# dmMaze/comic-text-detector

Hardware: NVIDIA H100
Metric: pages/sec @1024x1024 synthetic (higher is better)
Workload: dtype fp16

## Files before the change

### comic-text-detector_b200/csrc/engine.h

```cpp
#pragma once
#include <cuda.h>
#include <cuda_runtime.h>
#include <stdint.h>

#include <math.h>

#include <algorithm>
#include <array>
#include <condition_variable>
#include <deque>
#include <map>
#include <mutex>
#include <optional>
#include <string>
#include <thread>
#include <tuple>
#include <vector>

#include "kernels.h"

using ctd::ConvTcPlan;
using ctd::ConvEndsPlan;
using ctd::NmsWorkspace;
using ctd::PFN_encodeTiled;

struct ArenaLayout {
  size_t det, cnt, nl, lb, ls, lc, a_bytes, refined, blocks, blocks_stride, rec_off, lines_off, dist_off, total;
};

struct BlockSection {
  size_t rec_off, lines_off, dist_off, stride;
};
inline BlockSection block_section_layout() {
  auto al = [](size_t v) { return (v + 255) / 256 * 256; };
  BlockSection b;
  b.rec_off = 64;
  b.lines_off = b.rec_off + al(size_t(CTD_MAX_BLOCKS) * sizeof(ctd_block));
  b.dist_off = b.lines_off + al(size_t(CTD_MAX_BLOCKS) * 32);
  b.stride = b.dist_off + al(size_t(CTD_MAX_BLOCK_DIST) * 8);
  return b;
}

struct Letterbox {
  int unpad_h, unpad_w;
  float ratio_x, ratio_y;
};
inline bool letterbox_of(int ih, int iw, int net_h, int net_w, Letterbox& lb) {
  if (ih < 1 || iw < 1 || net_h < 1 || net_w < 1) return false;
  const double r = std::min(double(net_h) / ih, double(net_w) / iw);
  lb.unpad_w = int(nearbyint(iw * r));
  lb.unpad_h = int(nearbyint(ih * r));
  if (lb.unpad_w < 1 || lb.unpad_h < 1 || lb.unpad_w > net_w || lb.unpad_h > net_h) return false;
  lb.ratio_x = float(double(iw) / double(lb.unpad_w));
  lb.ratio_y = float(double(ih) / double(lb.unpad_h));
  return true;
}

struct PagesHead {
  size_t det, cnt, lb, ls, lc, masks;
};
PagesHead pages_head(int n);

struct JobPage {
  int ih, iw;
  float ratio_x, ratio_y;
  size_t off;
  char* section;
};

struct PipeJob {
  int slot = 0, refine_mode = 0;
  char* results_host = nullptr;
  PagesHead head{};
  size_t refined = 0;
  std::vector<JobPage> pages;
  size_t total = 0;
  const uint8_t* d_img = nullptr;
  uint8_t* d_mask = nullptr;
  uint8_t* d_ref = nullptr;
  uint8_t* d_aux = nullptr;
  uint8_t* d_blocks = nullptr;
  size_t blocks_bytes = 0;
  int keep_undetected = 0;
  int textheight = 0;
  int results_on_device = 0;
};

struct ctd_handle;
template <bool kPinned>
struct GrowBuf {
  uint8_t* p = nullptr;
  size_t cap = 0;
  int grow(ctd_handle* h, size_t bytes, std::optional<cudaStream_t> sync, size_t headroom = 4);
  void release();
};
using DevBuf = GrowBuf<false>;
using PinnedBuf = GrowBuf<true>;

struct Slot {
  uint8_t* d_stage_in = nullptr;
  uint8_t* d_stage_out = nullptr;
  cudaEvent_t ev_in_done = nullptr, ev_in_free = nullptr, ev_out_ready = nullptr, ev_out_done = nullptr;
  cudaEvent_t ev_post_done = nullptr;
  bool busy = false;
  bool full = false;
  bool crops = false, on_device = false, collected = false;
  int state = 0;
  int rc = 0;
  std::string err;
  char* pinned = nullptr;
  DevBuf pg_in, pg_res, pg_aux;
  ctd::PageGeom* h_pg_tab = nullptr;
  ctd::PageGeom* d_pg_tab = nullptr;
  std::vector<ctd_page_entry> dev_pages;
  std::vector<ctd_region> crop_plan;
  std::vector<int32_t> crop_first;
  std::vector<size_t> crop_base;
  DevBuf d_crop;
  PinnedBuf h_crop;
  size_t crop_px_off = 0, crop_bytes = 0;

  void start(bool want_crops, bool want_on_device) {
    crops = want_crops;
    on_device = want_on_device;
    collected = false;
  }
  void release();
};

struct RefineJob {
  std::vector<ctd::RefineWin> wins;
  std::vector<ctd::RefineChunk> chunks;
  size_t total_px = 0;
  void add(int x1, int y1, int x2, int y2, size_t page_off, int iw, int ih);
  size_t table_bytes() const;
};

struct RegionJob {
  std::vector<ctd::RegionDev> regs;
  std::vector<ctd::RegionTile> tiles;
  size_t out_bytes = 0;
  int add(const ctd_region* plan, int n, long long page_off, int ih, int iw, long long out_base);
  size_t table_bytes() const;
  void write_tables(char* dst) const;
};

struct ShapePlan {
  std::vector<ConvTcPlan> tc;
  std::vector<ConvEndsPlan> ends;
  cudaGraphExec_t graph = nullptr;
  int launches = 0;
};
struct ctd_handle {
  ctd_config cfg{};
  std::vector<ctd_op> ops;
  std::vector<ctd_bufdesc> bufs;
  std::vector<std::array<float, 7>> detect_prm;
  std::string err;
  cudaStream_t stream = nullptr;
  cudaEvent_t ev0 = nullptr, ev1 = nullptr, tev0 = nullptr, tev1 = nullptr;
  std::vector<cudaEvent_t> op_events;
  PFN_encodeTiled enc = nullptr;
  char* d_blob = nullptr;
  size_t blob_bytes = 0;
  std::vector<void*> d_buf;
  std::vector<void*> d_buf16;
  char* d_wsplit = nullptr;
  std::vector<size_t> wsplit_off;
  int elem = 2;
  uint8_t* d_pages = nullptr;
  float* d_blks = nullptr;
  float* d_mask = nullptr;
  uint8_t* d_mask_u8 = nullptr;
  size_t results_bytes = 0;
  float* d_lines = nullptr;
  uint8_t* d_bitmap = nullptr;
  float* d_det = nullptr;
  int* d_det_count = nullptr;
  int32_t* d_labels = nullptr;
  int32_t* d_nlabels = nullptr;
  int32_t* d_ccl_scratch = nullptr;
  void* d_segrep_scratch = nullptr;
  DevBuf refine_scratch;
  DevBuf cc_scratch;
  DevBuf io_scratch;
  int16_t* d_line_boxes = nullptr;
  float* d_line_scores = nullptr;
  int32_t* d_line_count = nullptr;
  void* d_nms_ws = nullptr;
  NmsWorkspace nms{};
  std::map<std::tuple<int, int, int>, ShapePlan> plans;
  cudaStream_t copy_in = nullptr, copy_out = nullptr;
  Slot slot[2];
  bool overlap = false;
  cudaStream_t side = nullptr, side2 = nullptr;
  cudaEvent_t ev_fork = nullptr, ev_join = nullptr, ev_fork2 = nullptr, ev_join2 = nullptr;
  cudaEvent_t ev_xjoin = nullptr;
  std::vector<char> db_ancestor;
  ArenaLayout layout{};
  cudaStream_t post = nullptr;
  size_t pipe_pinned_cap = 0;
  std::thread pipe_thread;
  std::mutex pipe_mu;
  std::condition_variable pipe_cv, pipe_done_cv;
  std::deque<PipeJob> pipe_queue;
  bool pipe_quit = false;
  int host_threads = 4;
  size_t pg_gather_off = 0;
  cudaStream_t dev_out = nullptr;
  DevBuf pg_cc;
  DevBuf post_refine;
  int n = 0, ph = 0, pw = 0;
  int last_launches = 0;
  bool have_forward = false;
};


int ctd_fail(ctd_handle* h, int code, const char* fmt, ...);
int prepare_forward(ctd_handle* h, int32_t n, int32_t ph, int32_t pw, ShapePlan** out);
int enqueue_forward(ctd_handle* h, int32_t n, int32_t ph, int32_t pw, ShapePlan& sp);
int ensure_pipeline(ctd_handle* h);
int stage_phase_a(ctd_handle* h, Slot& s, const uint8_t* pages, bool pages_on_device, int n, int ph, int pw,
                  ShapePlan& sp, void* results_host);
int cc_device(ctd_handle* h, const uint8_t* d_img, int ih, int iw, int stats_cap, int32_t** d_stats, int32_t* n_labels);
int launch_refine(ctd_handle* h, const RefineJob& job, const uint8_t* d_img, const uint8_t* d_mask, int refine_mode,
                  uint8_t* d_out, cudaStream_t st, DevBuf& scratch, char* pinned);
int ctd_collect_full(ctd_handle* h, int slot);
void ctd_pipeline_shutdown(ctd_handle* h);
```

### comic-text-detector_b200/csrc/kernels.h

```cpp
#pragma once
#include <cuda.h>
#include <cuda_fp16.h>
#include <cuda_runtime.h>
#include <stdint.h>

#include "../../include/ctd_b200.h"

namespace ctd {

constexpr int kMaxTaps = 9;

constexpr float kSplitLoScale = 2048.0f;
constexpr float kSplitLoUnscale = 1.0f / 2048.0f;
constexpr int kMaxPhases = 4;

struct ConvGeom {
  int n_img;
  int gh, gw;
  int dst_h, dst_w;
  int out_mul;
  int n_phase;
  int taps;
  int cin_total;
  int k_total;
  int n_src;
  int src_c[CTD_MAX_SRC];
  int src_cstride[CTD_MAX_SRC];
  int src_h, src_w;
  int in_stride;
  int8_t tap_dy[kMaxPhases][kMaxTaps];
  int8_t tap_dx[kMaxPhases][kMaxTaps];
  int cout, cout_pad;
  int dst_cstride, dst_coff;
  int act, residual;
};

void fill_conv_geom_taps(ConvGeom& g, int kind, int ksize, int stride);

struct alignas(64) ConvTcParams {
  CUtensorMap a_map[CTD_MAX_SRC][4];
  CUtensorMap b_map;
  CUtensorMap d_map[kMaxPhases];
  ConvGeom g;
  int kb_elems;
  int src_kblocks[CTD_MAX_SRC];
  int tiles_x, tiles_y;
  int8_t tap_map[kMaxPhases][kMaxTaps];
  __half* dst;
  int dst_map_cols;
  const float* bias;
  float* blks;
  int blks_rows_per_img;
  int level_row0;
  float det_stride;
  float anchor_wh[6];
  int nc;
  int split;
  int split_img_off;
  int split_row_off;
};
static_assert(sizeof(ConvTcParams) <= 4096, "ConvTcParams: kernel parameters are limited to 4 KB");

struct ConvTcPlan {
  ConvTcParams p;
  int block_n;
  int tile_h;
  dim3 grid;
  size_t smem_bytes;
};

typedef CUresult (*PFN_encodeTiled)(CUtensorMap*, CUtensorMapDataType, cuuint32_t, void*, const cuuint64_t*,
                                    const cuuint64_t*, const cuuint32_t*, const cuuint32_t*, CUtensorMapInterleave,
                                    CUtensorMapSwizzle, CUtensorMapL2promotion, CUtensorMapFloatOOBfill);

const char* conv_tc_plan(ConvTcPlan& plan, PFN_encodeTiled enc, const ConvGeom& g, const void* const src_ptr[],
                         const int src_coff[], const void* w16, const float* bias, __half* dst, int split = 0);
cudaError_t conv_tc_launch(const ConvTcPlan& plan, cudaStream_t s);
cudaError_t conv_tc_init();

enum { CTD_END_NONE = 0, CTD_END_STEM = 1, CTD_END_SEG = 2 };
struct alignas(64) ConvEndsParams {
  CUtensorMap a_map;
  CUtensorMap b_map;
  CUtensorMap d_map;
  int n_img, gh, gw;
  int tiles_x, tiles_y;
  const float* bias;
  float* mask_f32;
  uint8_t* mask_u8;
};
struct ConvEndsPlan {
  ConvEndsParams p;
  int kind = CTD_END_NONE;
  dim3 grid;
  size_t smem_bytes;
};
const char* conv_ends_plan_stem(ConvEndsPlan& plan, PFN_encodeTiled enc, const uint8_t* pages, int n, int ph, int pw,
                                const void* w16, const float* bias, __half* dst, int dst_cstride, int dst_coff,
                                int cout, int act);
const char* conv_ends_plan_seg(ConvEndsPlan& plan, PFN_encodeTiled enc, const __half* src, int src_cstride,
                               int src_coff, int src_c, int n, int gh, int gw, const void* w16, float* mask_f32,
                               uint8_t* mask_u8);
cudaError_t conv_ends_launch(const ConvEndsPlan& plan, cudaStream_t s);
cudaError_t conv_ends_init();

struct ConvSimtParams {
  ConvGeom g;
  const void* src[CTD_MAX_SRC];
  const void* w;
  const float* bias;
  void* dst;
  float* blks;
  int blks_rows_per_img, level_row0, nc;
  float det_stride;
  float anchor_wh[6];
};
template <typename T>
cudaError_t conv_simt_launch(const ConvSimtParams& p, cudaStream_t s);

template <typename T>
cudaError_t stem_launch(const uint8_t* pages, int n, int h, int w, const float* wgt ,
                        const float* bias, T* dst, int dst_cstride, int dst_coff, int cout, int act, cudaStream_t s);
cudaError_t split_planes_launch(const float* src, __half* hi, __half* lo, size_t npix, int c, int cstride,
                                cudaStream_t s);
template <typename T>
cudaError_t avgpool2_launch(const T* src, int n, int h, int w, int c, int src_cstride, T* dst, int dst_cstride,
                            cudaStream_t s);
template <typename T>
cudaError_t sppf_pool_launch(T* buf, int n, int h, int w, int c, int cstride, cudaStream_t s);
template <typename T>
cudaError_t upsample2_launch(const T* src, int n, int h, int w, int c, int src_cstride, T* dst, int dst_cstride,
                             cudaStream_t s);
template <typename T>
cudaError_t seg_tail_launch(const T* src, int n, int h, int w, int c, int cstride, const float* wgt ,
                            float* mask_f32, uint8_t* mask_u8, cudaStream_t s);
template <typename T>
cudaError_t db_tail_launch(const T* src, int n, int h, int w, int cstride, const float* params, float* lines,
                           uint8_t* bitmap, float db_thresh, cudaStream_t s);

struct NmsWorkspace {
  float* cand;
  int* cand_count;
  int* cand_total;
  float* sorted;
  unsigned long long* mask;
  int cap;
};
cudaError_t nms_launch(const float* blks, int n, int rows, int nc, float conf, float iou, NmsWorkspace& ws,
                       float* det , int* det_count, cudaStream_t s);
constexpr int kNmsLaunches = 5;
size_t nms_workspace_bytes(int n, int cap);
void nms_workspace_bind(NmsWorkspace& ws, void* base, int n, int cap);

cudaError_t ccl_launch(const uint8_t* img, int n, int h, int w, int32_t* labels, int32_t* scratch ,
                       int32_t* n_labels, cudaStream_t s);
constexpr int kCclLaunches = 8;
cudaError_t ccl_stats_launch(const int32_t* labels, int h, int w, int32_t* stats, int cap, cudaStream_t s);

size_t segrep_scratch_bytes(int n, int h, int w, int max_cand);
cudaError_t segrep_launch(const uint8_t* bitmap, const float* pred, size_t pred_page_stride, const int* Lf, int n, int h,
                          int w, int max_cand, float unclip_ratio, void* scratch, int16_t* boxes, float* scores,
                          int* n_contours, cudaStream_t s);
constexpr int kSegrepLaunches = 15;
cudaError_t binarize_launch(const float* pred, size_t count, float thresh, uint8_t* bitmap, cudaStream_t s);

cudaError_t resize_linear_u8_launch(const uint8_t* src, int sh, int sw, size_t src_pitch, int channels, uint8_t* dst,
                                    int dh, int dw, int canvas_h, int canvas_w, cudaStream_t s);
struct PageGeom {
  long long src_off, dst_off;
  int ih, iw, unpad_h, unpad_w, row0, pad;
};
cudaError_t letterbox_batch_launch(const uint8_t* src, const PageGeom* d_tab, int n, uint8_t* dst, int net_h, int net_w,
                                   cudaStream_t s);
cudaError_t backproject_batch_launch(const uint8_t* mask, int net_h, int net_w, const PageGeom* d_tab, int n,
                                     int total_rows, uint8_t* dst, cudaStream_t s);

struct GatherPage {
  const uint8_t* src;
  long long sh, sw, sc;
  long long dst_off;
  int ih, iw, row0, fast;
};
cudaError_t gather_pages_launch(const GatherPage* d_tab, int n, int total_rows, uint8_t* dst, cudaStream_t s);

struct RefineWin {
  int x1, y1, x2, y2;
  long long off;
  long long page_off;
  int pitch;
};
struct RefineChunk { int win, y0, x0, rows; };
constexpr int kRefineChunkPx = 8192;
__host__ __device__ constexpr int refine_rows_per_chunk(int rw) {
  return kRefineChunkPx / rw >= 8 ? (kRefineChunkPx / rw) & ~3 : (kRefineChunkPx / rw > 0 ? kRefineChunkPx / rw : 1);
}
size_t refine_scratch_bytes(size_t total_px, size_t n_chunks);
size_t refine_mk_state_bytes(int n_wins);
cudaError_t refine_mk_launch(const uint8_t* d_img, const uint8_t* d_mask, const RefineWin* d_wins, int n_wins,
                             const RefineChunk* d_chunks, int n_chunks, int n_multi_chunks, void* d_state, size_t total_px,
                             void* scratch, int refine_mode, uint8_t* d_out, cudaStream_t s);

constexpr int kRegionTilePx = 256;
struct RegionDev {
  long long offset;
  long long page_off;
  int out_h, out_w;
  int warp_w, bw0;
  int rotate, ih, iw, pad;
  double m[9];
};
struct RegionTile { int region, first; };
cudaError_t warp_regions_launch(const uint8_t* d_pages, const RegionDev* d_regs, const RegionTile* d_tiles, int n_tiles,
                                uint8_t* d_out, cudaStream_t s);

}
```

### comic-text-detector_b200/csrc/pipeline.cu

```cuda
#include <cuda.h>
#include <cuda_runtime.h>
#include <math.h>
#include <stdint.h>
#include <string.h>

#include <algorithm>
#include <thread>
#include <vector>

#include "engine.h"

using namespace ctd;

#define CK(expr)                                                                                      \
  do {                                                                                                \
    cudaError_t _e = (expr);                                                                          \
    if (_e != cudaSuccess) return ctd_fail(h, CTD_E_CUDA, "%s: %s (%s:%d)", #expr, cudaGetErrorString(_e), __FILE__, __LINE__); \
  } while (0)

namespace {
inline void norm_slice(int& lo, int& hi, int n) {
  if (lo < 0) lo = std::max(lo + n, 0);
  if (hi < 0) hi = std::max(hi + n, 0);
  lo = std::min(lo, n);
  hi = std::min(hi, n);
  if (hi < lo) hi = lo;
}
}

void RefineJob::add(int x1, int y1, int x2, int y2, size_t page_off, int iw, int ih) {
  norm_slice(x1, x2, iw);
  norm_slice(y1, y2, ih);
  const size_t a = (x2 > x1 && y2 > y1) ? size_t(x2 - x1) * (y2 - y1) : 0;
  if (a == 0) return;
  const int wi = int(wins.size());
  const int rw = x2 - x1, rh = y2 - y1;
  const int rows_per = refine_rows_per_chunk(rw);
  for (int y0 = 0; y0 < rh; y0 += rows_per)
    for (int x0 = 0; x0 < rw; x0 += kRefineChunkPx) chunks.push_back(RefineChunk{wi, y0, x0, std::min(rows_per, rh - y0)});
  wins.push_back(RefineWin{x1, y1, x2, y2, (long long)total_px, (long long)page_off, iw});
  total_px = (total_px + a + 3) / 4 * 4;
}
size_t RefineJob::table_bytes() const {
  auto al = [](size_t v) { return (v + 255) / 256 * 256; };
  return al(wins.size() * sizeof(RefineWin)) + al(chunks.size() * sizeof(RefineChunk));
}

int launch_refine(ctd_handle* h, const RefineJob& job, const uint8_t* d_img, const uint8_t* d_mask, int refine_mode,
                  uint8_t* d_out, cudaStream_t st, DevBuf& scratch, char* pinned) {
  if (job.wins.empty()) return CTD_OK;
  auto al = [](size_t v) { return (v + 255) / 256 * 256; };
  const size_t tb = job.table_bytes();
  const size_t sb = refine_mk_state_bytes(int(job.wins.size()));
  if (int rc = scratch.grow(h, tb + sb + refine_scratch_bytes(job.total_px, job.chunks.size()), st, 2)) return rc;
  char* base = reinterpret_cast<char*>(scratch.p);
  const size_t wb = al(job.wins.size() * sizeof(RefineWin));
  std::vector<char> local;
  char* stage = pinned;
  if (!stage) { local.resize(tb); stage = local.data(); }
  memcpy(stage, job.wins.data(), job.wins.size() * sizeof(RefineWin));
  int n_multi = 0;
  {
    RefineChunk* hc = reinterpret_cast<RefineChunk*>(stage + wb);
    const size_t nc = job.chunks.size();
    size_t tail = nc;
    for (size_t i = 0; i < nc;) {
      size_t j = i;
      while (j < nc && job.chunks[j].win == job.chunks[i].win) ++j;
      if (j - i > 1) {
        for (size_t k = i; k < j; ++k) hc[n_multi++] = job.chunks[k];
      } else {
        hc[--tail] = job.chunks[i];
      }
      i = j;
    }
  }
  CK(cudaMemcpyAsync(base, stage, tb, cudaMemcpyHostToDevice, st));
  if (!pinned) CK(cudaStreamSynchronize(st));
  CK(refine_mk_launch(d_img, d_mask, reinterpret_cast<const RefineWin*>(base), int(job.wins.size()),
                      reinterpret_cast<const RefineChunk*>(base + wb), int(job.chunks.size()), n_multi, base + tb,
                      job.total_px, base + tb + sb, refine_mode, d_out, st));
  return CTD_OK;
}

extern "C" int ctd_refine_mask(ctd_handle* h, const uint8_t* img, const uint8_t* mask, int32_t ih, int32_t iw,
                               const int32_t* windows, int32_t n_win, int32_t refine_mode, uint8_t* out) {
  if (!h || !img || !mask || !out || (n_win > 0 && !windows)) return CTD_E_INVALID;
  if (ih < 1 || iw < 1) return ctd_fail(h, CTD_E_SHAPE, "bad image size");
  CK(cudaSetDevice(h->cfg.device));
  RefineJob job;
  for (int i = 0; i < n_win; ++i) job.add(windows[4 * i], windows[4 * i + 1], windows[4 * i + 2], windows[4 * i + 3], 0, iw, ih);
  const size_t px = size_t(ih) * iw, pxa = (px + 255) / 256 * 256;
  if (int rc = h->io_scratch.grow(h, pxa * 5 + 1024, h->stream)) return rc;
  uint8_t* d_img = h->io_scratch.p;
  uint8_t* d_mask = d_img + pxa * 3;
  uint8_t* d_out = d_mask + pxa;
  CK(cudaMemcpyAsync(d_img, img, px * 3, cudaMemcpyHostToDevice, h->stream));
  CK(cudaMemcpyAsync(d_mask, mask, px, cudaMemcpyHostToDevice, h->stream));
  CK(cudaMemsetAsync(d_out, 0, pxa, h->stream));
  if (int rc = launch_refine(h, job, d_img, d_mask, refine_mode, d_out, h->stream, h->refine_scratch, nullptr))
    return rc;
  CK(cudaMemcpyAsync(out, d_out, px, cudaMemcpyDeviceToHost, h->stream));
  CK(cudaStreamSynchronize(h->stream));
  return CTD_OK;
}

namespace {
struct PageIn {
  const float* det; int n_det;
  const int16_t* line_boxes; const float* line_scores; int n_lines;
  const uint8_t* mask; int im_w, im_h;
  float ratio_x, ratio_y;
};

PageIn page_in(const char* res, const PagesHead& head, int i, const JobPage& p, const uint8_t* mask) {
  PageIn in;
  in.det = reinterpret_cast<const float*>(res + head.det) + size_t(i) * 300 * 6;
  in.n_det = std::min(std::max(reinterpret_cast<const int32_t*>(res + head.cnt)[i], 0), 300);
  in.line_boxes = reinterpret_cast<const int16_t*>(res + head.lb) + size_t(i) * 1000 * 8;
  in.line_scores = reinterpret_cast<const float*>(res + head.ls) + size_t(i) * 1000;
  in.n_lines = std::min(std::max(reinterpret_cast<const int32_t*>(res + head.lc)[i], 0), 1000);
  in.mask = mask; in.im_w = p.iw; in.im_h = p.ih; in.ratio_x = p.ratio_x; in.ratio_y = p.ratio_y;
  return in;
}

int host_group_page(const PageIn& in, char* section, const BlockSection& L, std::vector<int32_t>& win_out) {
  std::vector<int32_t> bxy(size_t(in.n_det) * 4), bcls(size_t(in.n_det));
  for (int i = 0; i < in.n_det; ++i) {
    const float* d = in.det + 6 * i;
    bxy[4 * i + 0] = int32_t(d[0] * in.ratio_x);
    bxy[4 * i + 1] = int32_t(d[1] * in.ratio_y);
    bxy[4 * i + 2] = int32_t(d[2] * in.ratio_x);
    bxy[4 * i + 3] = int32_t(d[3] * in.ratio_y);
    bcls[i] = int32_t(d[5]);
  }
  std::vector<int32_t> lines;
  lines.reserve(size_t(in.n_lines) * 8);
  for (int i = 0; i < in.n_lines; ++i) {
    if (!(in.line_scores[i] > 0.6f)) continue;
    const int16_t* b = in.line_boxes + 8 * i;
    for (int k = 0; k < 4; ++k) {
      lines.push_back(int32_t(double(b[2 * k]) * double(in.ratio_x)));
      lines.push_back(int32_t(double(b[2 * k + 1]) * double(in.ratio_y)));
    }
  }
  ctd_page_blocks* hdr = reinterpret_cast<ctd_page_blocks*>(section);
  ctd_block* rec = reinterpret_cast<ctd_block*>(section + L.rec_off);
  int32_t* lout = reinterpret_cast<int32_t*>(section + L.lines_off);
  double* dout = reinterpret_cast<double*>(section + L.dist_off);
  int32_t nb = 0;
  int rc = ctd_group_output(bxy.data(), bcls.data(), in.n_det, lines.data(), int32_t(lines.size() / 8), in.im_w, in.im_h, in.mask,
                            1, rec, CTD_MAX_BLOCKS, lout, CTD_MAX_BLOCKS, dout, CTD_MAX_BLOCK_DIST, &nb);
  hdr->flags = 0;
  if (rc == CTD_E_CAPACITY) {
    std::vector<double> big(size_t(CTD_MAX_BLOCKS) * CTD_MAX_BLOCKS / 4);
    rc = ctd_group_output(bxy.data(), bcls.data(), in.n_det, lines.data(), int32_t(lines.size() / 8), in.im_w, in.im_h, in.mask, 1,
                          rec, CTD_MAX_BLOCKS, lout, CTD_MAX_BLOCKS, big.data(), int32_t(big.size()), &nb);
    if (rc == CTD_OK)
      for (int i = 0; i < nb; ++i) { rec[i].n_dist = 0; rec[i].dist_off = 0; }
    hdr->flags |= 1;
  }
  if (rc != CTD_OK) { hdr->n_blocks = 0; hdr->n_lines = 0; hdr->n_dist = 0; hdr->flags |= 2; return rc; }
  hdr->n_blocks = nb;
  int32_t tl = 0, td = 0;
  for (int i = 0; i < nb; ++i) { tl += rec[i].n_lines; td += rec[i].n_dist; }
  hdr->n_lines = tl;
  hdr->n_dist = td;
  win_out.resize(size_t(nb) * 4);
  for (int i = 0; i < nb; ++i) {
    const int32_t* xy = rec[i].xyxy;
    const int64_t w = int64_t(xy[2]) - xy[0], hh = int64_t(xy[3]) - xy[1];
    const int64_t pad = int64_t(nearbyint((double(std::max(hh, w)) * 0.25 + double(std::min(hh, w)) * 0.75) / 16.0));
    win_out[4 * i + 0] = int32_t(std::max<int64_t>(0, xy[0] - pad));
    win_out[4 * i + 1] = int32_t(std::max<int64_t>(0, xy[1] - pad));
    win_out[4 * i + 2] = int32_t(std::min<int64_t>(in.im_w - 1, xy[2] + pad));
    win_out[4 * i + 3] = int32_t(std::min<int64_t>(in.im_h - 1, xy[3] + pad));
  }
  return CTD_OK;
}

template <typename F>
void for_each_page(int n, int threads, F fn) {
  const int nthreads = std::max(1, std::min(n, threads));
  if (nthreads == 1) {
    for (int i = 0; i < n; ++i) fn(i);
    return;
  }
  std::vector<std::thread> th;
  for (int t = 0; t < nthreads; ++t)
    th.emplace_back([&, t] { for (int i = t; i < n; i += nthreads) fn(i); });
  for (auto& x : th) x.join();
}

__global__ void undetected_prep_kernel(uint8_t* __restrict__ mask, const uint8_t* __restrict__ refined,
                                       uint8_t* __restrict__ thr, size_t n) {
  const size_t i = blockIdx.x * size_t(blockDim.x) + threadIdx.x;
  if (i >= n) return;
  uint8_t m = mask[i];
  if (refined[i] > 30) { m = 0; mask[i] = 0; }
  thr[i] = m > 30 ? 255 : 0;
}
__global__ void or_kernel(uint8_t* __restrict__ dst, const uint8_t* __restrict__ src, size_t n) {
  const size_t i = blockIdx.x * size_t(blockDim.x) + threadIdx.x;
  if (i < n) dst[i] |= src[i];
}

struct Planes {
  const uint8_t* img;
  uint8_t *mask, *ref, *ref2, *thr;
  size_t total;
};

int refine_undetected(ctd_handle* h, const std::vector<JobPage>& pages, const Planes& pl, int refine_mode,
                      cudaStream_t st, DevBuf& cc, DevBuf& refine_scratch, char* pinned, size_t pinned_cap) {
  auto al = [](size_t v) { return (v + 255) / 256 * 256; };
  const int n = int(pages.size());
  const size_t total_px = pl.total;
  undetected_prep_kernel<<<unsigned((total_px + 255) / 256), 256, 0, st>>>(pl.mask, pl.ref, pl.thr, total_px);
  CK(cudaGetLastError());
  size_t max_px = 0;
  std::vector<int> cap(static_cast<size_t>(n));
  std::vector<size_t> stats_off(static_cast<size_t>(n));
  for (int i = 0; i < n; ++i) max_px = std::max(max_px, size_t(pages[i].ih) * pages[i].iw);
  const size_t o_scr = al(max_px * 4);
  size_t o = o_scr + al(max_px * 12);
  for (int i = 0; i < n; ++i) {
    cap[size_t(i)] = ((pages[i].ih + 1) / 2) * ((pages[i].iw + 1) / 2) + 2;
    stats_off[size_t(i)] = o;
    o += al(size_t(cap[size_t(i)]) * 5 * 4);
  }
  const size_t o_nl = o;
  if (int rc = cc.grow(h, o_nl + al(size_t(n) * 4), st)) return rc;
  uint8_t* base = cc.p;
  int32_t* d_labels = reinterpret_cast<int32_t*>(base);
  int32_t* d_scr = reinterpret_cast<int32_t*>(base + o_scr);
  int32_t* d_nl = reinterpret_cast<int32_t*>(base + o_nl);
  for (int i = 0; i < n; ++i) {
    const JobPage& p = pages[size_t(i)];
    int32_t* d_stats = reinterpret_cast<int32_t*>(base + stats_off[size_t(i)]);
    CK(ccl_launch(pl.thr + p.off, 1, p.ih, p.iw, d_labels, d_scr, d_nl + i, st));
    CK(ccl_stats_launch(d_labels, p.ih, p.iw, d_stats, cap[size_t(i)], st));
  }
  std::vector<int32_t> n_lab(static_cast<size_t>(n));
  CK(cudaMemcpyAsync(n_lab.data(), d_nl, size_t(n) * 4, cudaMemcpyDeviceToHost, st));
  CK(cudaStreamSynchronize(st));
  std::vector<std::vector<int32_t>> stats(static_cast<size_t>(n));
  for (int i = 0; i < n; ++i) {
    stats[size_t(i)].resize(size_t(std::max(n_lab[size_t(i)], 0)) * 5);
    if (n_lab[size_t(i)] > 0)
      CK(cudaMemcpyAsync(stats[size_t(i)].data(), base + stats_off[size_t(i)], stats[size_t(i)].size() * 4,
                         cudaMemcpyDeviceToHost, st));
  }
  CK(cudaStreamSynchronize(st));
  const BlockSection bs = block_section_layout();
  RefineJob rj2;
  for (int i = 0; i < n; ++i) {
    const JobPage& p = pages[size_t(i)];
    const int nb = reinterpret_cast<const ctd_page_blocks*>(p.section)->n_blocks;
    const ctd_block* rec = reinterpret_cast<const ctd_block*>(p.section + bs.rec_off);
    bool first_valid = true;
    for (int li = 0; li < n_lab[size_t(i)]; ++li) {
      const int32_t* s5 = &stats[size_t(i)][size_t(li) * 5];
      if (!(s5[4] > 50)) continue;
      if (first_valid) { first_valid = false; continue; }
      const int64_t bb[4] = {s5[0], s5[1], int64_t(s5[0]) + s5[2], int64_t(s5[1]) + s5[3]};
      int64_t score = -1;
      for (int b = 0; b < nb; ++b) {
        const int32_t* q = rec[b].xyxy;
        const int64_t x1 = std::max<int64_t>(q[0], bb[0]), y1 = std::max<int64_t>(q[1], bb[1]);
        const int64_t x2 = std::min<int64_t>(q[2], bb[2]), y2 = std::min<int64_t>(q[3], bb[3]);
        const int64_t a = (y2 < y1 || x2 < x1) ? -1 : (y2 - y1) * (x2 - x1);
        if (a > score) score = a;
      }
      if (double(score) / double(s5[2]) / double(s5[3]) < 0.5) {
        int32_t xy[4] = {int32_t(bb[0]), int32_t(bb[1]), int32_t(bb[2]), int32_t(bb[3])}, w4[4];
        const int64_t w = bb[2] - bb[0], hh = bb[3] - bb[1];
        const int64_t pad = int64_t(nearbyint((double(std::max(hh, w)) * 0.25 + double(std::min(hh, w)) * 0.75) / 16.0));
        w4[0] = int32_t(std::max<int64_t>(0, xy[0] - pad)); w4[1] = int32_t(std::max<int64_t>(0, xy[1] - pad));
        w4[2] = int32_t(std::min<int64_t>(p.iw - 1, xy[2] + pad)); w4[3] = int32_t(std::min<int64_t>(p.ih - 1, xy[3] + pad));
        rj2.add(w4[0], w4[1], w4[2], w4[3], p.off, p.iw, p.ih);
      }
    }
  }
  if (!rj2.wins.empty()) {
    CK(cudaMemsetAsync(pl.ref2, 0, total_px, st));
    char* stage = rj2.table_bytes() <= pinned_cap ? pinned : nullptr;
    if (int rc = launch_refine(h, rj2, pl.img, pl.mask, refine_mode, pl.ref2, st, refine_scratch, stage)) return rc;
    or_kernel<<<unsigned((total_px + 255) / 256), 256, 0, st>>>(pl.ref, pl.ref2, total_px);
    CK(cudaGetLastError());
  }
  return CTD_OK;
}

int phase_c(ctd_handle* h, const std::vector<JobPage>& pages, const std::vector<std::vector<int32_t>>& wins,
            const Planes& pl, int refine_mode, bool keep_undetected, cudaStream_t st, DevBuf& refine_scratch,
            DevBuf& cc, char* pinned, size_t pinned_cap) {
  RefineJob rj;
  for (size_t i = 0; i < pages.size(); ++i)
    for (size_t k = 0; k + 3 < wins[i].size(); k += 4)
      rj.add(wins[i][k], wins[i][k + 1], wins[i][k + 2], wins[i][k + 3], pages[i].off, pages[i].iw, pages[i].ih);
  char* stage = rj.table_bytes() <= pinned_cap ? pinned : nullptr;
  if (int rc = launch_refine(h, rj, pl.img, pl.mask, refine_mode, pl.ref, st, refine_scratch, stage)) return rc;
  if (!keep_undetected) return CTD_OK;
  return refine_undetected(h, pages, pl, refine_mode, st, cc, refine_scratch, pinned, pinned_cap);
}
}

extern "C" int ctd_results_layout(ctd_handle* h, ctd_results_layout_t* out) {
  if (!h || !out) return CTD_E_INVALID;
  const ArenaLayout& L = h->layout;
  out->max_batch = h->cfg.max_batch; out->max_h = h->cfg.max_h; out->max_w = h->cfg.max_w; out->reserved = 0;
  out->total_bytes = L.total;
  out->mask_u8 = 0; out->det = L.det; out->det_count = L.cnt; out->n_labels = L.nl;
  out->line_boxes = L.lb; out->line_scores = L.ls; out->line_count = L.lc;
  out->phase_a_bytes = L.a_bytes;
  out->mask_refined = L.refined; out->blocks = L.blocks; out->blocks_stride = L.blocks_stride;
  out->blk_records_off = L.rec_off; out->blk_lines_off = L.lines_off; out->blk_dist_off = L.dist_off;
  return CTD_OK;
}

PagesHead pages_head(int n) {
  auto al = [](size_t v) { return (v + 255) / 256 * 256; };
  const size_t nb = size_t(n);
  PagesHead hd;
  hd.det = 0;
  hd.cnt = hd.det + al(nb * 300 * 6 * 4);
  hd.lb = hd.cnt + al(nb * 4);
  hd.ls = hd.lb + al(nb * 1000 * 8 * 2);
  hd.lc = hd.ls + al(nb * 1000 * 4);
  hd.masks = hd.lc + al(nb * 4);
  return hd;
}

extern "C" int ctd_pages_plan(ctd_page_entry* pages, int32_t n, int32_t net_h, int32_t net_w, size_t* input_bytes,
                              size_t* results_bytes) {
  if (!input_bytes || !results_bytes || n < 0 || (n > 0 && !pages)) return CTD_E_INVALID;
  if (net_h < 64 || net_w < 64 || net_h % 64 || net_w % 64) return CTD_E_SHAPE;
  auto al = [](size_t v) { return (v + 255) / 256 * 256; };
  const PagesHead hd = pages_head(n);
  size_t total = 0;
  for (int i = 0; i < n; ++i) {
    Letterbox lb;
    if (!letterbox_of(pages[i].ih, pages[i].iw, net_h, net_w, lb)) return CTD_E_SHAPE;
    pages[i].unpad_h = lb.unpad_h;
    pages[i].unpad_w = lb.unpad_w;
    pages[i].page_off = int64_t(total * 3);
    pages[i].mask_off = int64_t(hd.masks + total);
    total += al(size_t(pages[i].ih) * size_t(pages[i].iw));
  }
  const size_t stride = al(block_section_layout().stride);
  const size_t blocks = hd.masks + 2 * total;
  for (int i = 0; i < n; ++i) {
    pages[i].refined_off = pages[i].mask_off + int64_t(total);
    pages[i].blocks_off = int64_t(blocks + size_t(i) * stride);
  }
  *input_bytes = total * 3;
  *results_bytes = blocks + size_t(n) * stride;
  return CTD_OK;
}

static int plan_page_regions(const char* section, const BlockSection& bs, int iw, int ih, int textheight,
                             std::vector<ctd_region>& plan, size_t* bytes) {
  const ctd_page_blocks* hdr = reinterpret_cast<const ctd_page_blocks*>(section);
  const ctd_block* rec = reinterpret_cast<const ctd_block*>(section + bs.rec_off);
  const int32_t* quads = reinterpret_cast<const int32_t*>(section + bs.lines_off);
  std::vector<ctd_region_line> lines;
  lines.reserve(size_t(std::max(hdr->n_lines, 0)));
  for (int b = 0; b < hdr->n_blocks; ++b)
    for (int k = 0; k < rec[b].n_lines; ++k) {
      ctd_region_line l{};
      const int32_t* q = quads + size_t(rec[b].line_off + k) * 8;
      for (int j = 0; j < 8; ++j) l.quad[j] = double(q[j]);
      l.language = rec[b].language;
      l.vertical = rec[b].vertical ? 1 : 0;
      l.font_size = rec[b].font_size;
      lines.push_back(l);
    }
  plan.resize(lines.size());
  *bytes = 0;
  if (lines.empty()) return CTD_OK;
  return ctd_region_plan(lines.data(), int32_t(lines.size()), iw, ih, textheight, plan.data(), bytes);
}

static int run_batch(ctd_handle* h, const PipeJob& job) {
  Slot& s = h->slot[job.slot];
  const int n = int(job.pages.size());
  CK(cudaEventSynchronize(s.ev_out_done));
  char* res = job.results_host;
  const BlockSection bs = block_section_layout();
  std::vector<std::vector<int32_t>> wins(static_cast<size_t>(n));
  std::vector<int> prc(size_t(n), CTD_OK);
  const bool crops = job.textheight > 0;
  std::vector<std::vector<ctd_region>> plans(crops ? size_t(n) : 0);
  std::vector<size_t> plan_bytes(size_t(n), 0);
  std::vector<int> crc(size_t(n), CTD_OK);
  for_each_page(n, h->host_threads, [&](int i) {
    const JobPage& p = job.pages[size_t(i)];
    const uint8_t* mask = reinterpret_cast<const uint8_t*>(res + job.head.masks + p.off);
    prc[size_t(i)] = host_group_page(page_in(res, job.head, i, p, mask), p.section, bs, wins[size_t(i)]);
    if (crops && prc[size_t(i)] == CTD_OK)
      crc[size_t(i)] = plan_page_regions(p.section, bs, p.iw, p.ih, job.textheight, plans[size_t(i)],
                                         &plan_bytes[size_t(i)]);
  });
  for (int i = 0; i < n; ++i)
    if (prc[size_t(i)] != CTD_OK) return ctd_fail(h, prc[size_t(i)], "group_output failed on page %d of the batch", i);
  for (int i = 0; i < n; ++i)
    if (crc[size_t(i)] != CTD_OK)
      return ctd_fail(h, crc[size_t(i)], "ctd_region_plan refused page %d of the batch (%dx%d, textheight %d)", i,
                      job.pages[size_t(i)].ih, job.pages[size_t(i)].iw, job.textheight);
  RegionJob rg;
  if (crops) {
    s.crop_plan.clear();
    s.crop_first.assign(size_t(n) + 1, 0);
    s.crop_base.assign(size_t(n) + 1, 0);
    size_t base = 0;
    for (int i = 0; i < n; ++i) {
      const JobPage& pg = job.pages[size_t(i)];
      const std::vector<ctd_region>& p = plans[size_t(i)];
      if (int bad = rg.add(p.data(), int(p.size()), (long long)(pg.off * 3), pg.ih, pg.iw, (long long)base); bad >= 0)
        return ctd_fail(h, CTD_E_INVALID, "malformed crop plan entry %d on page %d of the batch", bad, i);
      s.crop_first[size_t(i)] = int32_t(s.crop_plan.size());
      s.crop_base[size_t(i)] = base;
      for (ctd_region r : p) {
        r.offset += int64_t(base);
        s.crop_plan.push_back(r);
      }
      base += plan_bytes[size_t(i)];
    }
    s.crop_first[size_t(n)] = int32_t(s.crop_plan.size());
    s.crop_base[size_t(n)] = base;
    if (s.crop_plan.size() > size_t(INT32_MAX) || rg.tiles.size() > size_t(INT32_MAX))
      return ctd_fail(h, CTD_E_CAPACITY, "too many crops in one batch");
    s.crop_bytes = base;
    s.crop_px_off = 0;
  }
  cudaStream_t st = h->post;
  CK(cudaStreamWaitEvent(st, s.ev_out_ready, 0));
  if (job.d_blocks)
    CK(cudaMemcpyAsync(job.d_blocks, job.pages[0].section, job.blocks_bytes, cudaMemcpyHostToDevice, st));
  const bool to_host = !job.results_on_device;
  if (!rg.tiles.empty()) {
    const size_t tb = rg.table_bytes(), px = s.crop_bytes;
    if (int rc = s.d_crop.grow(h, tb + px, st)) return rc;
    if (int rc = s.h_crop.grow(h, to_host ? tb + px : tb, st)) return rc;
    uint8_t* d_tab = s.d_crop.p;
    rg.write_tables(reinterpret_cast<char*>(s.h_crop.p));
    CK(cudaMemcpyAsync(d_tab, s.h_crop.p, tb, cudaMemcpyHostToDevice, st));
    const size_t rb = (rg.regs.size() * sizeof(ctd::RegionDev) + 255) / 256 * 256;
    CK(ctd::warp_regions_launch(job.d_img, reinterpret_cast<const ctd::RegionDev*>(d_tab),
                                reinterpret_cast<const ctd::RegionTile*>(d_tab + rb), int(rg.tiles.size()), d_tab + tb,
                                st));
    if (to_host) CK(cudaMemcpyAsync(s.h_crop.p + tb, d_tab + tb, px, cudaMemcpyDeviceToHost, st));
    s.crop_px_off = tb;
  }
  CK(cudaMemsetAsync(job.d_ref, 0, job.total, st));
  const Planes pl{job.d_img, job.d_mask, job.d_ref, job.d_aux, job.d_aux ? job.d_aux + job.total : nullptr, job.total};
  if (int rc = phase_c(h, job.pages, wins, pl, job.refine_mode, job.keep_undetected, st, h->post_refine, h->pg_cc,
                       s.pinned, h->pipe_pinned_cap))
    return rc;
  if (to_host) {
    if (job.keep_undetected) CK(cudaMemcpyAsync(res + job.head.masks, job.d_mask, job.total, cudaMemcpyDeviceToHost, st));
    CK(cudaMemcpyAsync(res + job.refined, job.d_ref, job.total, cudaMemcpyDeviceToHost, st));
  }
  CK(cudaEventRecord(s.ev_post_done, st));
  return CTD_OK;
}

static void pipe_worker(ctd_handle* h) {
  cudaSetDevice(h->cfg.device);
  for (;;) {
    PipeJob job;
    {
      std::unique_lock<std::mutex> lk(h->pipe_mu);
      h->pipe_cv.wait(lk, [&] { return h->pipe_quit || !h->pipe_queue.empty(); });
      if (h->pipe_queue.empty()) return;
      job = std::move(h->pipe_queue.front());
      h->pipe_queue.pop_front();
    }
    const int rc = run_batch(h, job);
    std::string err;
    if (rc != CTD_OK) err = h->err;
    {
      std::lock_guard<std::mutex> lk(h->pipe_mu);
      Slot& s = h->slot[job.slot];
      s.state = rc == CTD_OK ? 2 : 3;
      s.rc = rc;
      s.err = err;
    }
    h->pipe_done_cv.notify_all();
  }
}

static void queue_job(ctd_handle* h, PipeJob&& job) {
  Slot& s = h->slot[job.slot];
  {
    std::lock_guard<std::mutex> lk(h->pipe_mu);
    s.state = 1;
    h->pipe_queue.push_back(std::move(job));
  }
  h->pipe_cv.notify_one();
  s.busy = true;
  s.full = true;
}

static int ensure_full_pipeline(ctd_handle* h) {
  if (int rc = ensure_pipeline(h)) return rc;
  if (h->pipe_thread.joinable()) return CTD_OK;
  int lo = 0, hi = 0;
  CK(cudaDeviceGetStreamPriorityRange(&lo, &hi));
  CK(cudaStreamCreateWithPriority(&h->post, cudaStreamNonBlocking, hi));
  h->pipe_pinned_cap = size_t(h->cfg.max_batch) * (size_t(CTD_MAX_BLOCKS) * sizeof(RefineWin) +
                                                   size_t(CTD_MAX_BLOCKS) * sizeof(RefineChunk) * 8) + (size_t(8) << 20);
  for (Slot& s : h->slot) {
    CK(cudaHostAlloc(reinterpret_cast<void**>(&s.pinned), h->pipe_pinned_cap, cudaHostAllocDefault));
    CK(cudaEventCreateWithFlags(&s.ev_post_done, cudaEventDisableTiming));
  }
  const char* ht = getenv("CTD_HOST_THREADS");
  const unsigned hc = std::thread::hardware_concurrency();
  h->host_threads = ht ? atoi(ht) : int(std::max(1u, std::min(8u, hc ? hc / 2 : 4u)));
  h->pipe_quit = false;
  h->pipe_thread = std::thread(pipe_worker, h);
  return CTD_OK;
}

void ctd_pipeline_shutdown(ctd_handle* h) {
  if (h->pipe_thread.joinable()) {
    {
      std::lock_guard<std::mutex> lk(h->pipe_mu);
      h->pipe_quit = true;
    }
    h->pipe_cv.notify_all();
    h->pipe_thread.join();
  }
  if (h->post) cudaStreamDestroy(h->post);
  h->post = nullptr;
  if (h->dev_out) cudaStreamDestroy(h->dev_out);
  h->dev_out = nullptr;
  h->pg_cc.release();
  h->post_refine.release();
}

extern "C" int ctd_submit_full(ctd_handle* h, int32_t slot, const uint8_t* pages, int32_t n, int32_t ph, int32_t pw,
                               int32_t pages_on_device, int32_t refine_mode, void* results_host) {
  if (!h || !pages || !results_host || slot < 0 || slot > 1) return CTD_E_INVALID;
  if (h->cfg.debug_skip_postproc) return ctd_fail(h, CTD_E_INVALID, "ctd_submit_full needs the full pipeline");
  Slot& s = h->slot[slot];
  if (s.busy) return ctd_fail(h, CTD_E_INVALID, "slot %d has an uncollected submission", slot);
  ShapePlan* sp = nullptr;
  if (int rc = prepare_forward(h, n, ph, pw, &sp)) return rc;
  if (int rc = ensure_full_pipeline(h)) return rc;
  s.start(false, false);
  if (int rc = stage_phase_a(h, s, pages, pages_on_device != 0, n, ph, pw, *sp, results_host)) return rc;
  CK(cudaStreamWaitEvent(h->post, s.ev_out_ready, 0));
  const ArenaLayout& L = h->layout;
  const size_t px = size_t(ph) * pw;
  PipeJob job;
  job.slot = slot; job.refine_mode = refine_mode;
  job.results_host = static_cast<char*>(results_host);
  job.head = PagesHead{L.det, L.cnt, L.lb, L.ls, L.lc, 0};
  job.refined = L.refined;
  for (int i = 0; i < n; ++i)
    job.pages.push_back(JobPage{ph, pw, 1.f, 1.f, size_t(i) * px, job.results_host + L.blocks + size_t(i) * L.blocks_stride});
  job.total = size_t(n) * px;
  job.d_img = pages_on_device ? pages : s.d_stage_in;
  job.d_mask = s.d_stage_out;
  job.d_ref = s.d_stage_out + L.refined;
  job.d_blocks = s.d_stage_out + L.blocks;
  job.blocks_bytes = size_t(n) * L.blocks_stride;
  queue_job(h, std::move(job));
  return CTD_OK;
}

extern "C" int ctd_submit_pages(ctd_handle* h, int32_t slot, const ctd_page_entry* pages, int32_t n, int32_t net_h,
                                int32_t net_w, const uint8_t* input_host, int32_t refine_mode, int32_t keep_undetected,
                                void* results_host) {
  return ctd_submit_pages_regions(h, slot, pages, n, net_h, net_w, input_host, refine_mode, keep_undetected, 0,
                                  results_host);
}

extern "C" int ctd_submit_pages_regions(ctd_handle* h, int32_t slot, const ctd_page_entry* pages, int32_t n,
                                        int32_t net_h, int32_t net_w, const uint8_t* input_host, int32_t refine_mode,
                                        int32_t keep_undetected, int32_t textheight, void* results_host) {
  if (!input_host) return CTD_E_INVALID;
  return ctd_submit_pages_device(h, slot, pages, n, net_h, net_w, input_host, nullptr, refine_mode, keep_undetected,
                                 textheight, 0, results_host);
}

static bool is_device_memory(const void* p, int device) {
  cudaPointerAttributes a{};
  if (cudaPointerGetAttributes(&a, p) != cudaSuccess) {
    cudaGetLastError();
    return false;
  }
  return a.type == cudaMemoryTypeDevice && a.device == device;
}

extern "C" int ctd_submit_pages_device(ctd_handle* h, int32_t slot, const ctd_page_entry* pages, int32_t n,
                                       int32_t net_h, int32_t net_w, const uint8_t* input_host,
                                       const ctd_device_page* dev, int32_t refine_mode, int32_t keep_undetected,
                                       int32_t textheight, int32_t results_on_device, void* results_host) {
  if (!h || !pages || !results_host || slot < 0 || slot > 1 || n < 1) return CTD_E_INVALID;
  if (textheight != 0 && textheight < 2) return ctd_fail(h, CTD_E_INVALID, "textheight %d < 2", textheight);
  if (h->cfg.debug_skip_postproc) return ctd_fail(h, CTD_E_INVALID, "ctd_submit_pages needs the full pipeline");
  Slot& s = h->slot[slot];
  if (s.busy) return ctd_fail(h, CTD_E_INVALID, "slot %d has an uncollected submission", slot);
  if (n > h->cfg.max_batch) return ctd_fail(h, CTD_E_CAPACITY, "batch %d exceeds max_batch %d", n, h->cfg.max_batch);
  std::vector<ctd_page_entry> pg(pages, pages + n);
  size_t in_bytes = 0, res_bytes = 0;
  if (int rc = ctd_pages_plan(pg.data(), n, net_h, net_w, &in_bytes, &res_bytes))
    return ctd_fail(h, rc, "the pages do not letterbox into a %dx%d net input", net_h, net_w);
  if (memcmp(pg.data(), pages, size_t(n) * sizeof(ctd_page_entry)) != 0)
    return ctd_fail(h, CTD_E_INVALID, "the page entries are not the ones ctd_pages_plan returns");
  size_t rows = 0;
  for (int i = 0; i < n; ++i) rows += size_t(pg[size_t(i)].ih);
  if (rows > size_t(INT32_MAX)) return ctd_fail(h, CTD_E_CAPACITY, "the pages of a batch have more than 2^31 rows");
  CK(cudaSetDevice(h->cfg.device));
  int n_dev = 0;
  for (int i = 0; i < n; ++i) {
    if (!dev || !dev[i].data) {
      if (!input_host) return ctd_fail(h, CTD_E_INVALID, "page %d is in neither input_host nor device memory", i);
      continue;
    }
    const ctd_device_page& d = dev[i];
    const int64_t kMaxStride = int64_t(1) << 31;
    if (d.stride_h < 0 || d.stride_w < 0 || d.stride_c < 0 || d.stride_h > kMaxStride || d.stride_w > kMaxStride ||
        d.stride_c > kMaxStride)
      return ctd_fail(h, CTD_E_INVALID, "page %d: strides (%lld, %lld, %lld) out of range [0, 2^31]", i,
                      (long long)d.stride_h, (long long)d.stride_w, (long long)d.stride_c);
    const ctd_page_entry& e = pg[size_t(i)];
    const uint8_t* last = d.data + (e.ih - 1) * d.stride_h + (e.iw - 1) * d.stride_w + 2 * d.stride_c;
    if (!is_device_memory(d.data, h->cfg.device) || !is_device_memory(last, h->cfg.device))
      return ctd_fail(h, CTD_E_INVALID, "page %d (%p) is not device memory of GPU %d", i, (const void*)d.data,
                      h->cfg.device);
    ++n_dev;
  }
  ShapePlan* sp = nullptr;
  if (int rc = prepare_forward(h, n, net_h, net_w, &sp)) return rc;
  if (int rc = ensure_full_pipeline(h)) return rc;
  const ArenaLayout& L = h->layout;
  const PagesHead hd = pages_head(n);
  const size_t total = size_t(pg[0].refined_off - pg[0].mask_off);
  const size_t d2h = size_t(pg[0].refined_off);
  s.start(textheight > 0, results_on_device != 0);
  if (int rc = s.pg_in.grow(h, in_bytes, std::nullopt)) return rc;
  if (int rc = s.pg_res.grow(h, d2h + total, std::nullopt)) return rc;
  if (keep_undetected)
    if (int rc = s.pg_aux.grow(h, 2 * total, std::nullopt)) return rc;
  if (!s.h_pg_tab) {
    h->pg_gather_off = (size_t(h->cfg.max_batch) * sizeof(PageGeom) + 255) / 256 * 256;
    const size_t tab_bytes = h->pg_gather_off + size_t(h->cfg.max_batch) * sizeof(GatherPage);
    CK(cudaHostAlloc(reinterpret_cast<void**>(&s.h_pg_tab), tab_bytes, cudaHostAllocDefault));
    CK(cudaMalloc(reinterpret_cast<void**>(&s.d_pg_tab), tab_bytes));
  }
  PageGeom* tab = s.h_pg_tab;
  GatherPage* gtab = reinterpret_cast<GatherPage*>(reinterpret_cast<char*>(tab) + h->pg_gather_off);
  int row0 = 0, n_gather = 0, gather_rows = 0;
  for (int i = 0; i < n; ++i) {
    const ctd_page_entry& e = pg[size_t(i)];
    tab[i] = PageGeom{e.page_off, e.mask_off - int64_t(hd.masks), e.ih, e.iw, e.unpad_h, e.unpad_w, row0, 0};
    row0 += e.ih;
    if (dev && dev[i].data) {
      const ctd_device_page& d = dev[i];
      gtab[n_gather++] = GatherPage{d.data, (long long)d.stride_h, (long long)d.stride_w, (long long)d.stride_c,
                                    (long long)e.page_off, e.ih, e.iw, gather_rows,
                                    d.stride_c == 1 && d.stride_w == 3 ? 1 : 0};
      gather_rows += e.ih;
    }
  }
  const size_t tab_bytes = n_gather ? h->pg_gather_off + size_t(n_gather) * sizeof(GatherPage) : size_t(n) * sizeof(PageGeom);
  CK(cudaMemcpyAsync(s.d_pg_tab, tab, tab_bytes, cudaMemcpyHostToDevice, h->copy_in));
  if (n_dev == 0) {
    CK(cudaMemcpyAsync(s.pg_in.p, input_host, in_bytes, cudaMemcpyHostToDevice, h->copy_in));
  } else {
    for (int i = 0; i < n;) {
      if (dev[i].data) { ++i; continue; }
      int j = i;
      while (j + 1 < n && !dev[j + 1].data) ++j;
      const size_t lo = size_t(pg[size_t(i)].page_off);
      const size_t hi = size_t(pg[size_t(j)].page_off) + size_t(pg[size_t(j)].ih) * size_t(pg[size_t(j)].iw) * 3;
      CK(cudaMemcpyAsync(s.pg_in.p + lo, input_host + lo, hi - lo, cudaMemcpyHostToDevice, h->copy_in));
      i = j + 1;
    }
  }
  CK(cudaEventRecord(s.ev_in_done, h->copy_in));
  CK(cudaEventRecord(h->ev0, h->stream));
  CK(cudaStreamWaitEvent(h->stream, s.ev_in_done, 0));
  if (n_gather) {
    for (int i = 0; i < n; ++i)
      if (dev[i].data && dev[i].event) CK(cudaStreamWaitEvent(h->stream, static_cast<cudaEvent_t>(dev[i].event), 0));
    CK(gather_pages_launch(reinterpret_cast<const GatherPage*>(reinterpret_cast<const char*>(s.d_pg_tab) +
                                                               h->pg_gather_off),
                           n_gather, gather_rows, s.pg_in.p, h->stream));
  }
  CK(letterbox_batch_launch(s.pg_in.p, s.d_pg_tab, n, h->d_pages, net_h, net_w, h->stream));
  if (int rc = enqueue_forward(h, n, net_h, net_w, *sp)) return rc;
  uint8_t* d_res = s.pg_res.p;
  CK(backproject_batch_launch(h->d_mask_u8, net_h, net_w, s.d_pg_tab, n, row0, d_res + hd.masks, h->stream));
  const size_t nb = size_t(n);
  CK(cudaMemcpyAsync(d_res + hd.det, h->d_mask_u8 + L.det, nb * 300 * 6 * 4, cudaMemcpyDeviceToDevice, h->stream));
  CK(cudaMemcpyAsync(d_res + hd.cnt, h->d_mask_u8 + L.cnt, nb * 4, cudaMemcpyDeviceToDevice, h->stream));
  CK(cudaMemcpyAsync(d_res + hd.lb, h->d_mask_u8 + L.lb, nb * 1000 * 8 * 2, cudaMemcpyDeviceToDevice, h->stream));
  CK(cudaMemcpyAsync(d_res + hd.ls, h->d_mask_u8 + L.ls, nb * 1000 * 4, cudaMemcpyDeviceToDevice, h->stream));
  CK(cudaMemcpyAsync(d_res + hd.lc, h->d_mask_u8 + L.lc, nb * 4, cudaMemcpyDeviceToDevice, h->stream));
  CK(cudaEventRecord(s.ev_out_ready, h->stream));
  CK(cudaStreamWaitEvent(h->copy_out, s.ev_out_ready, 0));
  CK(cudaMemcpyAsync(results_host, d_res, d2h, cudaMemcpyDeviceToHost, h->copy_out));
  CK(cudaEventRecord(s.ev_out_done, h->copy_out));
  PipeJob job;
  job.slot = slot; job.refine_mode = refine_mode;
  job.results_host = static_cast<char*>(results_host);
  job.head = hd;
  job.refined = size_t(pg[0].refined_off);
  for (const ctd_page_entry& e : pg) {
    Letterbox lb;
    letterbox_of(e.ih, e.iw, net_h, net_w, lb);
    job.pages.push_back(JobPage{e.ih, e.iw, lb.ratio_x, lb.ratio_y, size_t(e.mask_off) - hd.masks,
                                job.results_host + e.blocks_off});
  }
  job.total = total;
  job.d_img = s.pg_in.p;
  job.d_mask = d_res + hd.masks;
  job.d_ref = d_res + pg[0].refined_off;
  job.d_aux = keep_undetected ? s.pg_aux.p : nullptr;
  job.keep_undetected = keep_undetected ? 1 : 0;
  job.textheight = textheight;
  job.results_on_device = results_on_device ? 1 : 0;
  if (results_on_device) s.dev_pages = std::move(pg);
  queue_job(h, std::move(job));
  return CTD_OK;
}

int ctd_collect_full(ctd_handle* h, int slot) {
  Slot& s = h->slot[slot];
  int rc;
  {
    std::unique_lock<std::mutex> lk(h->pipe_mu);
    h->pipe_done_cv.wait(lk, [&] { return s.state >= 2; });
    rc = s.rc;
    if (rc != CTD_OK) h->err = s.err;
    s.state = 0;
  }
  s.full = false;
  if (rc != CTD_OK) return rc;
  CK(cudaEventSynchronize(s.ev_post_done));
  s.collected = true;
  return CTD_OK;
}

extern "C" int ctd_collect_device(ctd_handle* h, int32_t slot, void* const* page_dst) {
  if (!h || slot < 0 || slot > 1 || !page_dst) return CTD_E_INVALID;
  const Slot& s = h->slot[slot];
  if (s.busy || !s.collected || !s.on_device)
    return ctd_fail(h, CTD_E_INVALID, "slot %d holds no collected batch with results on the device", slot);
  CK(cudaSetDevice(h->cfg.device));
  const std::vector<ctd_page_entry>& pg = s.dev_pages;
  const int n = int(pg.size());
  for (int i = 0; i < n; ++i)
    if (!page_dst[i] || !is_device_memory(page_dst[i], h->cfg.device))
      return ctd_fail(h, CTD_E_INVALID, "page_dst[%d] (%p) is not device memory of GPU %d", i, page_dst[i],
                      h->cfg.device);
  if (!h->dev_out) CK(cudaStreamCreateWithFlags(&h->dev_out, cudaStreamNonBlocking));
  const uint8_t* d_res = s.pg_res.p;
  const uint8_t* d_px = s.crops ? s.d_crop.p + s.crop_px_off : nullptr;
  for (int i = 0; i < n; ++i) {
    const ctd_page_entry& e = pg[size_t(i)];
    const size_t px = size_t(e.ih) * size_t(e.iw);
    uint8_t* dst = static_cast<uint8_t*>(page_dst[i]);
    CK(cudaMemcpyAsync(dst, d_res + e.mask_off, px, cudaMemcpyDeviceToDevice, h->dev_out));
    CK(cudaMemcpyAsync(dst + px, d_res + e.refined_off, px, cudaMemcpyDeviceToDevice, h->dev_out));
    if (s.crops) {
      const size_t b0 = s.crop_base[size_t(i)], b1 = s.crop_base[size_t(i) + 1];
      if (b1 > b0) CK(cudaMemcpyAsync(dst + 2 * px, d_px + b0, b1 - b0, cudaMemcpyDeviceToDevice, h->dev_out));
    }
  }
  CK(cudaStreamSynchronize(h->dev_out));
  return CTD_OK;
}

extern "C" int ctd_collect_regions(ctd_handle* h, int32_t slot, const ctd_region** plan, int32_t* n_regions,
                                   const int32_t** page_first, const uint8_t** pixels, size_t* bytes) {
  if (!h || slot < 0 || slot > 1 || !plan || !n_regions || !page_first || !pixels || !bytes) return CTD_E_INVALID;
  const Slot& s = h->slot[slot];
  if (s.busy || !s.collected || !s.crops)
    return ctd_fail(h, CTD_E_INVALID, "slot %d holds no collected ctd_submit_pages_regions batch", slot);
  *plan = s.crop_plan.data();
  *n_regions = int32_t(s.crop_plan.size());
  *page_first = s.crop_first.data();
  *bytes = s.crop_bytes;
  *pixels = s.crop_bytes && !s.on_device ? s.h_crop.p + s.crop_px_off : nullptr;
  return CTD_OK;
}

extern "C" int ctd_device_arena(ctd_handle* h, int32_t slot, void** base, void** post_stream) {
  if (!h || slot < 0 || slot > 1 || !base) return CTD_E_INVALID;
  if (!h->slot[slot].d_stage_out)
    return ctd_fail(h, CTD_E_INVALID, "no pipelined submission has been made on this handle");
  *base = h->slot[slot].d_stage_out;
  if (post_stream) *post_stream = h->post;
  return CTD_OK;
}

extern "C" int ctd_detect_page(ctd_handle* h, const uint8_t* page, int32_t ih, int32_t iw, int32_t net_h, int32_t net_w,
                               int32_t refine_mode, int32_t keep_undetected, uint8_t* mask_out, uint8_t* mask_refined_out,
                               ctd_block* blocks, int32_t blocks_cap, int32_t* lines_out, int32_t lines_cap, double* dist_out,
                               int32_t dist_cap, int32_t* n_blocks) {
  if (!h || !page || !mask_out || !mask_refined_out || !n_blocks) return CTD_E_INVALID;
  if (ih < 1 || iw < 1) return ctd_fail(h, CTD_E_SHAPE, "bad page size %dx%d", ih, iw);
  *n_blocks = 0;
  Letterbox geo;
  if (!letterbox_of(ih, iw, net_h, net_w, geo)) return ctd_fail(h, CTD_E_SHAPE, "page does not letterbox into the net input");
  ShapePlan* sp = nullptr;
  if (int rc = prepare_forward(h, 1, net_h, net_w, &sp)) return rc;
  const size_t px = size_t(ih) * iw, pxa = (px + 255) / 256 * 256;
  if (int rc = h->io_scratch.grow(h, pxa * 7 + 1024, h->stream)) return rc;
  uint8_t* d_page = h->io_scratch.p;
  uint8_t* d_mask = d_page + pxa * 3;
  uint8_t* d_ref = d_mask + pxa;
  uint8_t* d_ref2 = d_ref + pxa;
  uint8_t* d_thr = d_ref2 + pxa;
  cudaStream_t st = h->stream;
  CK(cudaEventRecord(h->ev0, st));
  CK(cudaMemcpyAsync(d_page, page, px * 3, cudaMemcpyHostToDevice, st));
  const bool same = ih == net_h && iw == net_w;
  if (same) CK(cudaMemcpyAsync(h->d_pages, d_page, px * 3, cudaMemcpyDeviceToDevice, st));
  else CK(resize_linear_u8_launch(d_page, ih, iw, size_t(iw) * 3, 3, h->d_pages, geo.unpad_h, geo.unpad_w, net_h, net_w, st));
  if (int rc = enqueue_forward(h, 1, net_h, net_w, *sp)) return rc;
  if (same) CK(cudaMemcpyAsync(d_mask, h->d_mask_u8, px, cudaMemcpyDeviceToDevice, st));
  else CK(resize_linear_u8_launch(h->d_mask_u8, geo.unpad_h, geo.unpad_w, size_t(net_w), 1, d_mask, ih, iw, ih, iw, st));
  const PagesHead hd = pages_head(1);
  std::vector<char> rows(hd.masks);
  CK(cudaMemcpyAsync(mask_out, d_mask, px, cudaMemcpyDeviceToHost, st));
  CK(cudaMemcpyAsync(rows.data() + hd.det, h->d_det, 300 * 6 * 4, cudaMemcpyDeviceToHost, st));
  CK(cudaMemcpyAsync(rows.data() + hd.cnt, h->d_det_count, 4, cudaMemcpyDeviceToHost, st));
  CK(cudaMemcpyAsync(rows.data() + hd.lb, h->d_line_boxes, 1000 * 8 * 2, cudaMemcpyDeviceToHost, st));
  CK(cudaMemcpyAsync(rows.data() + hd.ls, h->d_line_scores, 1000 * 4, cudaMemcpyDeviceToHost, st));
  CK(cudaMemcpyAsync(rows.data() + hd.lc, h->d_line_count, 4, cudaMemcpyDeviceToHost, st));
  CK(cudaMemsetAsync(d_ref, 0, pxa, st));
  CK(cudaStreamSynchronize(st));
  const BlockSection L = block_section_layout();
  std::vector<char> section(L.stride);
  const std::vector<JobPage> pages{JobPage{ih, iw, geo.ratio_x, geo.ratio_y, 0, section.data()}};
  std::vector<std::vector<int32_t>> wins(1);
  if (int rc = host_group_page(page_in(rows.data(), hd, 0, pages[0], mask_out), section.data(), L, wins[0]))
    return ctd_fail(h, rc, "group_output failed");
  const ctd_page_blocks* hdr = reinterpret_cast<const ctd_page_blocks*>(section.data());
  const ctd_block* rec = reinterpret_cast<const ctd_block*>(section.data() + L.rec_off);
  const int nb = hdr->n_blocks;
  *n_blocks = nb;
  if (nb > blocks_cap || hdr->n_lines > lines_cap || hdr->n_dist > dist_cap || (nb > 0 && (!blocks || !lines_out)) ||
      (hdr->n_dist > 0 && !dist_out))
    return ctd_fail(h, CTD_E_CAPACITY, "%d blocks / %d lines / %d distances do not fit the output arrays", nb, hdr->n_lines, hdr->n_dist);
  if (nb > 0) {
    memcpy(blocks, rec, size_t(nb) * sizeof(ctd_block));
    memcpy(lines_out, section.data() + L.lines_off, size_t(hdr->n_lines) * 32);
    if (hdr->n_dist > 0) memcpy(dist_out, section.data() + L.dist_off, size_t(hdr->n_dist) * 8);
  }
  const Planes pl{d_page, d_mask, d_ref, d_ref2, d_thr, px};
  if (int rc = phase_c(h, pages, wins, pl, refine_mode, keep_undetected, st, h->refine_scratch, h->cc_scratch, nullptr, 0))
    return rc;
  if (keep_undetected) CK(cudaMemcpyAsync(mask_out, d_mask, px, cudaMemcpyDeviceToHost, st));
  CK(cudaMemcpyAsync(mask_refined_out, d_ref, px, cudaMemcpyDeviceToHost, st));
  CK(cudaStreamSynchronize(st));
  return CTD_OK;
}
```

### comic-text-detector_b200/csrc/refine_mk.cu

```cuda
#include <cuda_runtime.h>
#include <limits.h>
#include <math.h>

#include "kernels.h"

namespace ctd {

namespace {

constexpr int kThreads = 256;
constexpr int kChunkPx = kRefineChunkPx;

struct WinState {
  int hist[4][256];
  unsigned long long xs[12];
  int lo[3], hi[3], otsu_t[3], ncol;
  int nproc, proc_kind[4], proc_neg[4];
  int area0, max1, cnt1, max2;
  int pad[2];
};

struct Ctx {
  const uint8_t* img_all;
  const uint8_t* mask_all;
  uint32_t* out_all;
  const RefineWin* wins;
  const RefineChunk* chunks;
  WinState* st;
  int mode;
  uint16_t* lab;
  uint16_t* roots;
  int* nroots;
  int* P;
  int* acc;
  uint8_t *grey, *predm, *merged, *tmp;
};
constexpr uint16_t kNoLabel = 0xffffu;
static_assert(kChunkPx <= 0xffff, "a chunk-local offset fits 16 bits below kNoLabel");

struct View {
  RefineWin win;
  int w, rw, rh, y0, x0, rows, cols, i0, cnt, aligned;
  const uint8_t* img;
  const uint8_t* mask;
};

__device__ __forceinline__ View view_of(const Ctx& c, int chunk) {
  View v;
  const RefineChunk ch = c.chunks[chunk];
  v.w = ch.win;
  v.win = c.wins[ch.win];
  v.rw = v.win.x2 - v.win.x1;
  v.rh = v.win.y2 - v.win.y1;
  v.y0 = ch.y0;
  v.x0 = ch.x0;
  v.rows = ch.rows;
  v.cols = min(v.rw - ch.x0, kChunkPx);
  v.i0 = ch.y0 * v.rw + ch.x0;
  v.cnt = ch.rows * v.cols;
  v.aligned = (v.i0 & 3) == 0;
  v.img = c.img_all + size_t(v.win.page_off) * 3;
  v.mask = c.mask_all + size_t(v.win.page_off);
  return v;
}

__device__ __forceinline__ int chunk_start(int y, int x, int rw) {
  if (rw > kChunkPx) return y * rw + (x & ~(kChunkPx - 1));
  const int rows_per = refine_rows_per_chunk(rw);
  return (y / rows_per) * rows_per * rw;
}
static_assert((kChunkPx & (kChunkPx - 1)) == 0, "row segments start on multiples of kChunkPx");

__device__ __forceinline__ int uf_find(const int* L, int a) {
  int p = __ldcg(L + a);
  while (p != a) {
    a = p;
    p = __ldcg(L + a);
  }
  return a;
}
__device__ __forceinline__ int uf_find_compress(int* L, int a) {
  const int r = uf_find(L, a);
  while (a != r) {
    const int p = __ldcg(L + a);
    if (p <= r) break;
    atomicMin(&L[a], r);
    a = p;
  }
  return r;
}
__device__ __forceinline__ void uf_union(int* L, int a, int b) {
  bool done;
  do {
    a = uf_find(L, a);
    b = uf_find(L, b);
    if (a < b) {
      const int old = atomicMin(&L[b], a);
      done = old == b;
      b = old;
    } else if (b < a) {
      const int old = atomicMin(&L[a], b);
      done = old == a;
      a = old;
    } else {
      done = true;
    }
  } while (!done);
}

__device__ __forceinline__ void hist_add(int* hist, int bin) {
  const int b0 = __shfl_sync(0xffffffffu, bin, 0);
  if (__all_sync(0xffffffffu, bin == b0)) {
    if ((threadIdx.x & 31) == 0 && bin >= 0) atomicAdd(&hist[bin], 32);
    return;
  }
  if (bin >= 0) atomicAdd(&hist[bin], 1);
}

struct DivW { int d; float inv; bool fast; };
__device__ __forceinline__ DivW make_div(int d, int n) { return DivW{d, __frcp_rn(float(d)), n < (1 << 24)}; }
__device__ __forceinline__ void divmod(int i, const DivW& dv, int& q, int& r) {
  if (dv.fast) {
    q = __float2int_rz(__int2float_rn(i) * dv.inv);
    r = i - q * dv.d;
    if (r < 0) { --q; r += dv.d; } else if (r >= dv.d) { ++q; r -= dv.d; }
  } else {
    q = i / dv.d;
    r = i - q * dv.d;
  }
}

constexpr int kU = 4;
constexpr int kExtWords = (3 * kChunkPx) / 32 + 4;
static_assert(3 * (kChunkPx + 2) / 32 + 2 < kExtWords, "a row segment's halo rectangle fits the shared bit masks");
struct Halo {
  int ystart, xs, ew, ext, off;
};
__device__ __forceinline__ Halo halo_of(const View& v) {
  Halo h;
  h.ystart = v.y0 > 0 ? v.y0 - 1 : 0;
  h.xs = v.x0 > 0 ? v.x0 - 1 : 0;
  h.ew = min(v.x0 + v.cols + 1, v.rw) - h.xs;
  h.ext = (min(v.y0 + v.rows + 1, v.rh) - h.ystart) * h.ew;
  h.off = (v.y0 - h.ystart) * h.ew + v.x0 - h.xs;
  return h;
}
__device__ __forceinline__ unsigned bits_from(const unsigned* M, int pos) {
  if (pos <= -32) return 0u;
  if (pos < 0) return M[0] << (-pos);
  const int w = pos >> 5, sft = pos & 31;
  return __funnelshift_r(M[w], M[w + 1], sft);
}
__device__ __forceinline__ void row_ends(int x, int rw, unsigned& rs, unsigned& re) {
  rs = 0u;
  for (int j = x == 0 ? 0 : rw - x; j < 32; j += rw) rs |= 1u << j;
  int xe = x + 32;
  if (xe >= rw) xe %= rw;
  re = (rs >> 1) | (xe == 0 ? 0x80000000u : 0u);
}
__global__ void __launch_bounds__(kThreads) k_phase0(Ctx c) {
  __shared__ int sh[4][256];
  __shared__ unsigned N60[kExtWords], N127[kExtWords];
  __shared__ unsigned F60[kChunkPx / 32 + 1], F127[kChunkPx / 32 + 1];
  const View v = view_of(c, blockIdx.x);
  for (int i = threadIdx.x; i < 1024; i += kThreads) (&sh[0][0])[i] = 0;
  for (int i = threadIdx.x; i < kExtWords; i += kThreads) { N60[i] = 0u; N127[i] = 0u; }
  __syncthreads();
  uint8_t* grey = c.grey + v.win.off;
  uint8_t* predm = c.predm + v.win.off;
  uint8_t* merged = c.merged + v.win.off;
  const Halo hl = halo_of(v);
  const DivW dv = make_div(hl.ew, 3 * (kChunkPx + 2) + 1);
  for (int e0 = 0; e0 < hl.ext; e0 += kThreads) {
    const int e = e0 + threadIdx.x;
    int mv = 255;
    if (e < hl.ext) {
      int ye, xe;
      divmod(e, dv, ye, xe);
      mv = v.mask[size_t(v.win.y1 + hl.ystart + ye) * v.win.pitch + v.win.x1 + hl.xs + xe];
    }
    const unsigned b60 = __ballot_sync(0xffffffffu, mv <= 60), b127 = __ballot_sync(0xffffffffu, mv <= 127);
    if ((threadIdx.x & 31) == 0 && e < hl.ext) { N60[e >> 5] = b60; N127[e >> 5] = b127; }
  }
  __syncthreads();
  const int ew = hl.ew;
  for (int w = threadIdx.x; w * 32 < v.cnt; w += kThreads) {
    const int p = w * 32 + hl.off;
    int ye, xe;
    divmod(p, dv, ye, xe);
    unsigned rs, re;
    row_ends(hl.xs + xe, v.rw, rs, re);
    F60[w] = bits_from(N60, p) | bits_from(N60, p - ew) | bits_from(N60, p + ew) | (bits_from(N60, p - 1) & ~rs) |
             (bits_from(N60, p + 1) & ~re);
    F127[w] = bits_from(N127, p) | bits_from(N127, p - ew) | bits_from(N127, p + ew) |
              ((bits_from(N127, p - 1) | bits_from(N127, p - ew - 1) | bits_from(N127, p + ew - 1)) & ~rs) |
              ((bits_from(N127, p + 1) | bits_from(N127, p - ew + 1) | bits_from(N127, p + ew + 1)) & ~re);
  }
  __syncthreads();
  const DivW dvw = make_div(v.rw, v.rw * v.rh);
  for (int k0 = 0; k0 < v.cnt; k0 += kThreads * kU) {
    int b[kU], g[kU], r[kU];
#pragma unroll
    for (int u = 0; u < kU; ++u) {
      const int k = k0 + u * kThreads + threadIdx.x;
      b[u] = -1; g[u] = -1; r[u] = -1;
      if (k < v.cnt) {
        int y, x;
        divmod(v.i0 + k, dvw, y, x);
        const size_t gp = size_t(v.win.y1 + y) * v.win.pitch + v.win.x1 + x;
        b[u] = v.img[gp * 3]; g[u] = v.img[gp * 3 + 1]; r[u] = v.img[gp * 3 + 2];
      }
    }
#pragma unroll
    for (int u = 0; u < kU; ++u) {
      const int k = k0 + u * kThreads + threadIdx.x;
      const bool in = k < v.cnt;
      int gr = 0;
      bool core = false;
      if (in) {
        const int i = v.i0 + k;
        gr = (b[u] * 1868 + g[u] * 9617 + r[u] * 4899 + 8192) >> 14;
        grey[i] = (uint8_t)gr;
        predm[i] = ((F60[k >> 5] >> (k & 31)) & 1u) ? 0 : 255;
        merged[i] = 0;
        core = !((F127[k >> 5] >> (k & 31)) & 1u);
      }
      if (k0 + u * kThreads < v.cnt) {
        hist_add(sh[1], b[u]);
        hist_add(sh[2], g[u]);
        hist_add(sh[3], r[u]);
        hist_add(sh[0], core ? gr : -1);
      }
    }
  }
  __syncthreads();
  int* gh = &c.st[v.w].hist[0][0];
  for (int i = threadIdx.x; i < 1024; i += kThreads) {
    const int val = (&sh[0][0])[i];
    if (val) atomicAdd(&gh[i], val);
  }
}

constexpr int kDecideThreads = 64;
__global__ void __launch_bounds__(kDecideThreads) k_decide1(Ctx c) {
  __shared__ int cnt255[256];
  __shared__ int order[256];
  __shared__ double edges[256];
  __shared__ int s_first, s_last, s_total;
  __shared__ int hist_s[4][256];
  WinState& st = c.st[blockIdx.x];
  const RefineWin win = c.wins[blockIdx.x];
  const int n = (win.x2 - win.x1) * (win.y2 - win.y1);
  for (int i = threadIdx.x; i < 1024; i += kDecideThreads) (&hist_s[0][0])[i] = (&st.hist[0][0])[i];
  const int* hist_g = hist_s[0];
  for (int i = threadIdx.x; i < 256; i += kDecideThreads) cnt255[i] = 0;
  __syncthreads();
  if (threadIdx.x == 0) {
    int first = -1, last = -1, total = 0;
    for (int v = 0; v < 256; ++v)
      if (hist_g[v]) { if (first < 0) first = v; last = v; total += hist_g[v]; }
    s_first = first; s_last = last; s_total = total;
  }
  __syncthreads();
  {
    double fe, le;
    if (s_total == 0) { fe = 0.0; le = 1.0; }
    else if (s_first == s_last) { fe = s_first - 0.5; le = s_last + 0.5; }
    else { fe = s_first; le = s_last; }
    const double step = (le - fe) / 255.0;
    for (int i = threadIdx.x; i < 256; i += kDecideThreads) edges[i] = (i == 255) ? le : __dadd_rn(__dmul_rn((double)i, step), fe);
    __syncthreads();
    for (int v = threadIdx.x; v < 256; v += kDecideThreads) {
      if (!hist_g[v]) continue;
      const double a = (double)v;
      const double f = ((a - fe) / (le - fe)) * 255.0;
      int idx = (int)f;
      if (idx == 255) idx = 254;
      if (a < edges[idx]) --idx;
      if (a >= edges[idx + 1] && idx != 254) ++idx;
      atomicAdd(&cnt255[idx], hist_g[v]);
    }
  }
  __syncthreads();
  for (int b = threadIdx.x; b < 255; b += kDecideThreads) {
    int rank = 0;
    const int cb = cnt255[b];
    for (int q = 0; q < 255; ++q) rank += (cnt255[q] > cb) || (cnt255[q] == cb && q < b);
    order[rank] = b;
  }
  __syncthreads();
  if (threadIdx.x == 0) {
    double top[3];
    int nt = 1;
    top[0] = edges[order[0]];
    const double tol = (double)s_total * 0.001;
    for (int j = 1; j < 255; ++j) {
      const double col = edges[order[j]];
      double dmin = 1e300;
      for (int t = 0; t < nt; ++t) dmin = fmin(dmin, fabs(top[t] - col));
      if (dmin > 10.0) top[nt++] = col;
      if (nt >= 3 || (double)cnt255[order[j]] < tol) break;
    }
    st.ncol = nt;
    for (int t = 0; t < nt; ++t) {
      const double c_top = fmin(top[t] + 30.0, 255.0);
      const double c_bot = c_top - 60.0;
      st.lo[t] = (int)fmin(fmax(rint(c_bot), 0.0), 255.0);
      st.hi[t] = (int)fmin(fmax(rint(c_top), 0.0), 255.0);
    }
  }
  if (threadIdx.x >= 32 && threadIdx.x < 35) {
    const int* hh = hist_s[1 + threadIdx.x - 32];
    const double scale = 1.0 / (double)n;
    double mu = 0;
    for (int i = 0; i < 256; ++i) mu = __dadd_rn(mu, __dmul_rn((double)i, (double)hh[i]));
    mu = __dmul_rn(mu, scale);
    double mu1 = 0, q1 = 0, max_sigma = 0;
    int max_val = 0;
    for (int i = 0; i < 256; ++i) {
      const double p_i = __dmul_rn((double)hh[i], scale);
      mu1 = __dmul_rn(mu1, q1);
      q1 = __dadd_rn(q1, p_i);
      const double q2 = 1.0 - q1;
      if (fmin(q1, q2) < 1.1920929e-07 || fmax(q1, q2) > 1.0 - 1.1920929e-07) continue;
      mu1 = __ddiv_rn(__dadd_rn(mu1, __dmul_rn((double)i, p_i)), q1);
      const double mu2 = __ddiv_rn(__dsub_rn(mu, __dmul_rn(q1, mu1)), q2);
      const double dm = __dsub_rn(mu1, mu2);
      const double sigma = __dmul_rn(__dmul_rn(__dmul_rn(q1, q2), dm), dm);
      if (sigma > max_sigma) { max_sigma = sigma; max_val = i; }
    }
    st.otsu_t[threadIdx.x - 32] = max_val;
  }
}

__global__ void __launch_bounds__(kThreads) k_xor(Ctx c) {
  __shared__ unsigned long long sx[12];
  const View v = view_of(c, blockIdx.x);
  const WinState& st = c.st[v.w];
  if (threadIdx.x < 12) sx[threadIdx.x] = 0ull;
  __syncthreads();
  const uint8_t* grey = c.grey + v.win.off;
  const int ncol = st.ncol;
  int lo[3], hi[3], ot[3];
#pragma unroll
  for (int k = 0; k < 3; ++k) { lo[k] = st.lo[k]; hi[k] = st.hi[k]; ot[k] = st.otsu_t[k]; }
  unsigned pos[6], npx = 0;
#pragma unroll
  for (int k = 0; k < 6; ++k) pos[k] = 0u;
  const DivW dv = make_div(v.rw, v.rw * v.rh);
  for (int k0 = 0; k0 < v.cnt; k0 += kThreads * kU) {
    int mk[kU], gr[kU], ch[kU][3];
#pragma unroll
    for (int u = 0; u < kU; ++u) {
      const int k = k0 + u * kThreads + threadIdx.x;
      mk[u] = -1;
      if (k < v.cnt) {
        int y, x;
        divmod(v.i0 + k, dv, y, x);
        const size_t gp = size_t(v.win.y1 + y) * v.win.pitch + v.win.x1 + x;
        mk[u] = v.mask[gp];
        gr[u] = grey[v.i0 + k];
#pragma unroll
        for (int q = 0; q < 3; ++q) ch[u][q] = v.img[gp * 3 + q];
      }
    }
#pragma unroll
    for (int u = 0; u < kU; ++u) {
      if (mk[u] < 0) continue;
      ++npx;
#pragma unroll
      for (int k = 0; k < 3; ++k) {
        const int t = (gr[u] >= lo[k] && gr[u] <= hi[k]) ? 255 : 0;
        pos[k] += (unsigned)(t ^ mk[u]);
        const int t2 = ch[u][k] > ot[k] ? 255 : 0;
        pos[3 + k] += (unsigned)(t2 ^ mk[u]);
      }
    }
  }
#pragma unroll
  for (int k = 0; k < 6; ++k) {
    const bool used = k >= 3 || k < ncol;
    unsigned long long sp = used ? pos[k] : 0ull, sn = used ? 255ull * npx - pos[k] : 0ull;
    for (int o = 16; o > 0; o >>= 1) {
      sp += __shfl_down_sync(0xffffffffu, sp, o);
      sn += __shfl_down_sync(0xffffffffu, sn, o);
    }
    if ((threadIdx.x & 31) == 0) {
      if (sp) atomicAdd(&sx[2 * k], sp);
      if (sn) atomicAdd(&sx[2 * k + 1], sn);
    }
  }
  __syncthreads();
  if (threadIdx.x < 12 && sx[threadIdx.x]) atomicAdd(&c.st[v.w].xs[threadIdx.x], sx[threadIdx.x]);
}

__global__ void k_decide2(Ctx c, int n_wins) {
  const int w = blockIdx.x * blockDim.x + threadIdx.x;
  if (w >= n_wins) return;
  WinState& st = c.st[w];
  const unsigned long long* xs = st.xs;
  unsigned long long best[4];
  int kind[4], neg[4], np_ = 0;
  for (int k = 0; k < st.ncol; ++k) {
    const bool ng = xs[2 * k + 1] < xs[2 * k];
    best[np_] = ng ? xs[2 * k + 1] : xs[2 * k];
    kind[np_] = k; neg[np_] = ng; ++np_;
  }
  int bc = 0, bneg = 0;
  unsigned long long bv = ~0ull;
  for (int ch = 0; ch < 3; ++ch) {
    const bool ng = xs[6 + 2 * ch + 1] < xs[6 + 2 * ch];
    const unsigned long long val = ng ? xs[6 + 2 * ch + 1] : xs[6 + 2 * ch];
    if (val < bv) { bv = val; bc = ch; bneg = ng; }
  }
  best[np_] = bv; kind[np_] = 3 + bc; neg[np_] = bneg; ++np_;
  for (int i = 1; i < np_; ++i) {
    const unsigned long long val = best[i];
    const int kk = kind[i], nn = neg[i];
    int j = i - 1;
    while (j >= 0 && best[j] > val) { best[j + 1] = best[j]; kind[j + 1] = kind[j]; neg[j + 1] = neg[j]; --j; }
    best[j + 1] = val; kind[j + 1] = kk; neg[j + 1] = nn;
  }
  for (int i = 0; i < np_; ++i) { st.proc_kind[i] = kind[i]; st.proc_neg[i] = neg[i]; }
  st.nproc = np_;
  st.area0 = 0; st.max1 = -1; st.cnt1 = 0; st.max2 = -1;
}

constexpr int kLabelThreads = 512;

__device__ __forceinline__ int suf_find(const int* L, int a) {
  int p = L[a];
  while (p != a) {
    a = p;
    p = L[a];
  }
  return a;
}
__device__ __forceinline__ int suf_find_halve(int* L, int a) {
  int p = L[a];
  while (p != a) {
    const int gp = L[p];
    if (gp != p) atomicMin(&L[a], gp);
    a = p;
    p = gp;
  }
  return a;
}
__device__ __forceinline__ void suf_union(int* L, int a, int b) {
  bool done;
  do {
    a = suf_find_halve(L, a);
    b = suf_find_halve(L, b);
    if (a < b) {
      const int old = atomicMin(&L[b], a);
      done = old == b;
      b = old;
    } else if (b < a) {
      const int old = atomicMin(&L[a], b);
      done = old == a;
      a = old;
    } else {
      done = true;
    }
  } while (!done);
}

__global__ void __launch_bounds__(kLabelThreads, 3) k_label_local(Ctx c, int round) {
  __shared__ int Ls[kChunkPx];
  __shared__ unsigned Mw[kChunkPx / 32 + 2];
  __shared__ unsigned Sw[kChunkPx / 32];
  __shared__ unsigned Gw[kChunkPx / 32];
  __shared__ unsigned Bw[kChunkPx / 32];
  __shared__ int s_fg, s_nroot;
  const View v = view_of(c, blockIdx.x);
  WinState& st = c.st[v.w];
  if (round < 4 && round >= st.nproc) return;
  for (int i = threadIdx.x; i < kChunkPx / 32 + 2; i += kLabelThreads) Mw[i] = 0u;
  if (threadIdx.x == 0) { s_fg = 0; s_nroot = 0; }
  __syncthreads();
  uint16_t* lab = c.lab + v.win.off + v.i0;
  uint16_t* roots = c.roots + v.win.off + v.i0;
  int* P = c.P + v.win.off;
  int* acc = c.acc + 4 * v.win.off;
  const int n = v.rw * v.rh;
  int* area = acc; int* gain = acc + n; int* loss = acc + 2 * n; int* maxi = acc + 3 * n;
  const uint8_t* grey = c.grey + v.win.off;
  const uint8_t* merged = c.merged + v.win.off;
  const uint8_t* predm = c.predm + v.win.off;
  int kind = 0, neg = 0, lo = 0, hi = 0, ot = 0;
  if (round < 4) {
    kind = st.proc_kind[round]; neg = st.proc_neg[round];
    if (kind < 3) { lo = st.lo[kind]; hi = st.hi[kind]; } else ot = st.otsu_t[kind - 3];
  }
  const int lane = threadIdx.x & 31;
  const DivW dv = make_div(v.rw, kChunkPx + 1);
  constexpr int kIt = kChunkPx / kLabelThreads;
  if (v.aligned) {
    const uint32_t* mg32 = reinterpret_cast<const uint32_t*>(merged + v.i0);
    const uint32_t* pd32 = reinterpret_cast<const uint32_t*>(predm + v.i0);
    const uint32_t* gr32 = reinterpret_cast<const uint32_t*>(grey + v.i0);
    const int sh = 4 * (lane & 7);
    const unsigned grp = 0xffu << (8 * (lane >> 3));
#pragma unroll 1
    for (int it = 0; it < kChunkPx / (4 * kLabelThreads); ++it) {
      if (it * 4 * kLabelThreads >= v.cnt) break;
      const int k = 4 * (it * kLabelThreads + int(threadIdx.x));
      unsigned fg4 = 0u, g4 = 0u, b4 = 0u;
      if (k < v.cnt) {
        const unsigned m4 = mg32[k >> 2], p4 = pd32[k >> 2];
        unsigned s4 = m4;
        if (round < 4) {
          if (kind < 3) {
            s4 = gr32[k >> 2];
          } else {
            s4 = 0u;
#pragma unroll
            for (int j = 0; j < 4; ++j) {
              if (k + j < v.cnt) {
                int yl, x;
                divmod(k + j, dv, yl, x);
                s4 |= unsigned(v.img[(size_t(v.win.y1 + v.y0 + yl) * v.win.pitch + v.win.x1 + v.x0 + x) * 3 + (kind - 3)]) << (8 * j);
              }
            }
          }
        }
#pragma unroll
        for (int j = 0; j < 4; ++j) {
          if (k + j < v.cnt) {
            const int sbv = int((s4 >> (8 * j)) & 0xffu), mb = int((m4 >> (8 * j)) & 0xffu), pb = int((p4 >> (8 * j)) & 0xffu);
            bool fg;
            if (round == 4) {
              fg = sbv == 0;
            } else {
              const bool t = kind < 3 ? (sbv >= lo && sbv <= hi) : (sbv > ot);
              fg = neg ? !t : t;
            }
            const bool un = fg && mb == 0;
            fg4 |= unsigned(fg) << j;
            g4 |= unsigned(un && pb != 0) << j;
            b4 |= unsigned(un && pb == 0) << j;
          }
        }
      }
      const unsigned M = __reduce_or_sync(grp, fg4 << sh), G = __reduce_or_sync(grp, g4 << sh), B = __reduce_or_sync(grp, b4 << sh);
      if ((lane & 7) == 0) { const int w = k >> 5; Mw[w] = M; Gw[w] = G; Bw[w] = B; }
    }
    __syncthreads();
    for (int w = threadIdx.x; w * 32 < v.cnt; w += kLabelThreads) {
      const unsigned M = Mw[w];
      int yl, x0;
      divmod(w * 32, dv, yl, x0);
      unsigned rs = 0u;
      for (int j = x0 == 0 ? 0 : v.rw - x0; j < 32; j += v.rw) rs |= 1u << j;
      const unsigned S = M & (~(M << 1) | rs);
      Sw[w] = S;
      unsigned f = S;
      while (f) {
        const int k = w * 32 + __ffs(f) - 1;
        f &= f - 1u;
        Ls[k] = k;
      }
    }
  } else {
    constexpr int kB = 4;
    int xrun, xstep;
    {
      int q;
      divmod(int(threadIdx.x), dv, q, xrun);
      divmod(kLabelThreads, dv, q, xstep);
    }
  #pragma unroll 1
    for (int ub = 0; ub < kIt; ub += kB) {
      if (ub * kLabelThreads >= v.cnt) break;
      int raw[kB], mg[kB], pd[kB];
  #pragma unroll
      for (int u = 0; u < kB; ++u) {
        const int k = (ub + u) * kLabelThreads + threadIdx.x;
        raw[u] = 0; mg[u] = 1; pd[u] = 0;
        if (k < v.cnt) {
          const int i = v.i0 + k;
          mg[u] = merged[i];
          pd[u] = predm[i];
          if (round == 4) raw[u] = mg[u];
          else if (kind < 3) raw[u] = grey[i];
          else {
            int yl, x;
            divmod(k, dv, yl, x);
            raw[u] = v.img[(size_t(v.win.y1 + v.y0 + yl) * v.win.pitch + v.win.x1 + v.x0 + x) * 3 + (kind - 3)];
          }
        }
      }
  #pragma unroll
      for (int u = 0; u < kB; ++u) {
        const int k0 = (ub + u) * kLabelThreads;
        if (k0 >= v.cnt) break;
        const int k = k0 + threadIdx.x;
        const bool in = k < v.cnt;
        int sv = 0;
        const int x = xrun;
        xrun += xstep;
        if (xrun >= v.rw) xrun -= v.rw;
        if (in) {
          if (round == 4) {
            sv = raw[u] ? 0 : 255;
          } else {
            const int tv = kind < 3 ? ((raw[u] >= lo && raw[u] <= hi) ? 255 : 0) : (raw[u] > ot ? 255 : 0);
            sv = neg ? 255 - tv : tv;
          }
        }
        const bool fg = in && sv != 0;
        const bool un = fg && mg[u] == 0;
        const unsigned m = __ballot_sync(0xffffffffu, fg);
        const unsigned gb = __ballot_sync(0xffffffffu, un && pd[u] != 0);
        const unsigned lb = __ballot_sync(0xffffffffu, un && pd[u] == 0);
        const bool starts = fg && (lane == 0 || x == 0 || !((m >> (lane - 1)) & 1u));
        const unsigned sb = __ballot_sync(0xffffffffu, starts);
        if (lane == 0) { Mw[k >> 5] = m; Sw[k >> 5] = sb; Gw[k >> 5] = gb; Bw[k >> 5] = lb; }
        if (starts) Ls[k] = k;
      }
    }
  }
  __syncthreads();
  auto start_of = [&](int pos) -> int {
    return (pos & ~31) + 31 - __clz(Sw[pos >> 5] & (0xffffffffu >> (31 - (pos & 31))));
  };
  auto bits_at = [&](int pos) -> unsigned {
    if (pos <= -32) return 0u;
    if (pos < 0) return Mw[0] << (-pos);
    const int w = pos >> 5, sft = pos & 31;
    return __funnelshift_r(Mw[w], Mw[w + 1], sft);
  };
  for (int hw = threadIdx.x; hw * 16 < v.cnt; hw += kLabelThreads) {
    const int w = hw >> 1;
    const unsigned half = (hw & 1) ? 0xffff0000u : 0x0000ffffu;
    const unsigned cur = Mw[w];
    if (!(cur & half)) continue;
    const int k0 = w * 32;
    int yl, x0;
    divmod(k0, dv, yl, x0);
    unsigned rs = 0u;
    for (int j = x0 == 0 ? 0 : v.rw - x0; j < 32; j += v.rw) rs |= 1u << j;
    int xe = x0 + 32;
    if (xe >= v.rw) xe %= v.rw;
    const unsigned re = (rs >> 1) | (xe == 0 ? 0x80000000u : 0u);
    const unsigned lft = bits_at(k0 - 1);
    if (!(hw & 1) && (cur & 1u) && !(rs & 1u) && (lft & 1u)) suf_union(Ls, k0, start_of(k0 - 1));
    if (k0 + 32 <= v.rw) continue;
    const unsigned vup = (k0 >= v.rw ? 0xffffffffu : (0xffffffffu << (v.rw - k0))) & half;
    const unsigned up = bits_at(k0 - v.rw), upl = bits_at(k0 - v.rw - 1), upr = bits_at(k0 - v.rw + 1);
    unsigned f = cur & up & vup & (rs | ~lft | ~upl);
    while (f) {
      const int j = __ffs(f) - 1;
      f &= f - 1u;
      suf_union(Ls, start_of(k0 + j), start_of(k0 + j - v.rw));
    }
    const unsigned nb = cur & ~up & vup;
    f = nb & upl & ~rs;
    while (f) {
      const int j = __ffs(f) - 1;
      f &= f - 1u;
      suf_union(Ls, start_of(k0 + j), start_of(k0 + j - v.rw - 1));
    }
    f = nb & upr & ~re;
    while (f) {
      const int j = __ffs(f) - 1;
      f &= f - 1u;
      suf_union(Ls, start_of(k0 + j), start_of(k0 + j - v.rw + 1));
    }
  }
  __syncthreads();
  int fgc = 0;
  for (int hw = threadIdx.x; hw * 16 < v.cnt; hw += kLabelThreads) {
    const unsigned half = (hw & 1) ? 0xffff0000u : 0x0000ffffu;
    unsigned f = Sw[hw >> 1] & half;
    fgc += __popc(Mw[hw >> 1] & half);
    const int k0 = (hw >> 1) * 32;
    while (f) {
      const int s0 = k0 + __ffs(f) - 1;
      f &= f - 1u;
      const int r = suf_find(Ls, s0);
      if (r != s0) {
        atomicMin(&Ls[s0], r);
      } else {
        const int gi = v.i0 + s0;
        area[gi] = 0; gain[gi] = 0; loss[gi] = 0; maxi[gi] = -1;
        P[gi] = gi;
        roots[atomicAdd(&s_nroot, 1)] = uint16_t(s0);
      }
    }
  }
  if (round == 4) {
    for (int o = 16; o > 0; o >>= 1) fgc += __shfl_down_sync(0xffffffffu, fgc, o);
    if (lane == 0 && fgc) atomicAdd(&s_fg, fgc);
  }
  __syncthreads();
  if (threadIdx.x == 0) {
    c.nroots[blockIdx.x] = s_nroot;
    const int a0 = v.cnt - s_fg;
    if (round == 4 && a0) atomicAdd(&st.area0, a0);
  }
  for (int k = threadIdx.x; k < v.cnt; k += kLabelThreads)
    lab[k] = ((Mw[k >> 5] >> (k & 31)) & 1u) ? uint16_t(Ls[start_of(k)]) : kNoLabel;
  for (int hw = threadIdx.x; hw * 16 < v.cnt; hw += kLabelThreads) {
    const int w = hw >> 1;
    const unsigned M = Mw[w], S = Sw[w];
    unsigned f = S & ((hw & 1) ? 0xffff0000u : 0x0000ffffu);
    if (!f) continue;
    const unsigned G = Gw[w], B = Bw[w];
    const int k0 = w * 32;
    while (f) {
      const int sbit = __ffs(f) - 1;
      f &= f - 1u;
      const unsigned stop = (~M | S) & (0xfffffffeu << sbit);
      const int e = stop ? __ffs(stop) - 2 : 31;
      const unsigned rm = (e == 31 ? 0xffffffffu : ((2u << e) - 1u)) & ~((1u << sbit) - 1u);
      const int gi = v.i0 + Ls[k0 + sbit];
      atomicAdd(&area[gi], __popc(rm));
      atomicMax(&maxi[gi], v.i0 + k0 + e);
      const int g_ = __popc(rm & G), l_ = __popc(rm & B);
      if (g_) atomicAdd(&gain[gi], g_);
      if (l_) atomicAdd(&loss[gi], l_);
    }
  }
}
constexpr int kBorderThreads = 256;
__global__ void __launch_bounds__(kBorderThreads) k_union_border(Ctx c, int round) {
  const View v = view_of(c, blockIdx.x);
  if (round < 4 && round >= c.st[v.w].nproc) return;
  if (v.i0 == 0) return;
  const uint16_t* lab = c.lab + v.win.off;
  int* P = c.P + v.win.off;
  auto root_at = [&](int y, int x) { const int i = y * v.rw + x; return chunk_start(y, x, v.rw) + lab[i]; };
  const int y = v.y0;
  if (v.x0 > 0 && threadIdx.x == 0 && lab[v.i0] != kNoLabel && lab[v.i0 - 1] != kNoLabel)
    uf_union(P, v.i0 + lab[v.i0], root_at(y, v.x0 - 1));
  if (y == 0) return;
  for (int k = threadIdx.x; k < v.cols; k += int(blockDim.x)) {
    const int i = v.i0 + k, x = v.x0 + k;
    if (lab[i] == kNoLabel) continue;
    const int up = i - v.rw;
    const int r = v.i0 + lab[i];
    if (lab[up] != kNoLabel) {
      const bool first = x == 0 || lab[i - 1] == kNoLabel || lab[up - 1] == kNoLabel;
      if (first) uf_union(P, r, root_at(y - 1, x));
    } else {
      if (x > 0 && lab[up - 1] != kNoLabel) uf_union(P, r, root_at(y - 1, x - 1));
      if (x + 1 < v.rw && lab[up + 1] != kNoLabel) uf_union(P, r, root_at(y - 1, x + 1));
    }
  }
}
__global__ void __launch_bounds__(kThreads) k_flat1(Ctx c, int round) {
  const View v = view_of(c, blockIdx.x);
  if (round < 4 && round >= c.st[v.w].nproc) return;
  const uint16_t* roots = c.roots + v.win.off + v.i0;
  const int nr = c.nroots[blockIdx.x];
  int* P = c.P + v.win.off;
  int* acc = c.acc + 4 * v.win.off;
  const int n = v.rw * v.rh;
  int* area = acc; int* gain = acc + n; int* loss = acc + 2 * n; int* maxi = acc + 3 * n;
  for (int j = threadIdx.x; j < nr; j += kThreads) {
    const int cr = v.i0 + roots[j];
    const int g = uf_find_compress(P, cr);
    if (g != cr) {
      atomicAdd(&area[g], area[cr]);
      atomicMax(&maxi[g], maxi[cr]);
      const int g_ = gain[cr], l_ = loss[cr];
      if (g_) atomicAdd(&gain[g], g_);
      if (l_) atomicAdd(&loss[g], l_);
    }
  }
}
__global__ void __launch_bounds__(kThreads) k_top_a(Ctx c) {
  const View v = view_of(c, blockIdx.x);
  WinState& st = c.st[v.w];
  const int* P = c.P + v.win.off;
  const int* area = c.acc + 4 * v.win.off;
  const uint16_t* roots = c.roots + v.win.off + v.i0;
  const int nr = c.nroots[blockIdx.x];
  int m = -1;
  for (int j = threadIdx.x; j < nr; j += kThreads) {
    const int i = v.i0 + roots[j];
    if (P[i] == i) m = max(m, area[i]);
  }
  if (v.i0 == 0 && threadIdx.x == 0) m = max(m, st.area0);
  for (int o = 16; o > 0; o >>= 1) m = max(m, __shfl_down_sync(0xffffffffu, m, o));
  if ((threadIdx.x & 31) == 0 && m >= 0) atomicMax(&st.max1, m);
}
__global__ void __launch_bounds__(kThreads) k_top_b(Ctx c) {
  const View v = view_of(c, blockIdx.x);
  WinState& st = c.st[v.w];
  const int* P = c.P + v.win.off;
  const int* area = c.acc + 4 * v.win.off;
  const uint16_t* roots = c.roots + v.win.off + v.i0;
  const int nr = c.nroots[blockIdx.x];
  const int m1 = st.max1;
  int m2 = -1, c1 = 0;
  auto push = [&](int a) { if (a == m1) ++c1; else m2 = max(m2, a); };
  for (int j = threadIdx.x; j < nr; j += kThreads) {
    const int i = v.i0 + roots[j];
    if (P[i] == i) push(area[i]);
  }
  if (v.i0 == 0 && threadIdx.x == 0) push(st.area0);
  for (int o = 16; o > 0; o >>= 1) {
    m2 = max(m2, __shfl_down_sync(0xffffffffu, m2, o));
    c1 += __shfl_down_sync(0xffffffffu, c1, o);
  }
  if ((threadIdx.x & 31) == 0) {
    if (c1) atomicAdd(&st.cnt1, c1);
    if (m2 >= 0) atomicMax(&st.max2, m2);
  }
}
__global__ void __launch_bounds__(kThreads) k_mapply(Ctx c, int round) {
  const View v = view_of(c, blockIdx.x);
  const WinState& st = c.st[v.w];
  if (round < 4 && round >= st.nproc) return;
  const uint16_t* lab = c.lab + v.win.off + v.i0;
  const int* P = c.P + v.win.off;
  uint8_t* merged = c.merged + v.win.off;
  const int* acc = c.acc + 4 * v.win.off;
  const int n = v.rw * v.rh;
  const int* area = acc; const int* gain = acc + n; const int* loss = acc + 2 * n; const int* maxi = acc + 3 * n;
  const int second = st.cnt1 >= 2 ? st.max1 : st.max2;
  const int thresh = second >= 0 ? second : st.max1;
  __shared__ uint8_t dec[kChunkPx];
  const uint16_t* roots = c.roots + v.win.off + v.i0;
  const int nr = c.nroots[blockIdx.x];
  for (int j = threadIdx.x; j < nr; j += kThreads) {
    const int cl = roots[j];
    const int g = P[v.i0 + cl];
    const int a = area[g];
    bool ok;
    if (round < 4) {
      const int mx = maxi[g];
      ok = !(a == 1 || (a == 2 && (mx == g + 1 || mx == g + v.rw)));
    } else {
      ok = a < thresh;
    }
    dec[cl] = ok && gain[g] > loss[g];
  }
  __syncthreads();
  auto merges = [&](unsigned l) { return l != kNoLabel && dec[l]; };
  int k_tail = 0;
  if (v.aligned) {
    const uint2* lab4 = reinterpret_cast<const uint2*>(lab);
    uint32_t* mg32 = reinterpret_cast<uint32_t*>(merged + v.i0);
    const int n4 = v.cnt >> 2;
    for (int q = threadIdx.x; q < n4; q += kThreads) {
      const uint2 l4 = lab4[q];
      const unsigned m = (merges(l4.x & 0xffffu) ? 0xffu : 0u) | (merges(l4.x >> 16) ? 0xff00u : 0u) |
                         (merges(l4.y & 0xffffu) ? 0xff0000u : 0u) | (merges(l4.y >> 16) ? 0xff000000u : 0u);
      if (m) mg32[q] |= m;
    }
    k_tail = n4 << 2;
  }
  for (int k = k_tail + threadIdx.x; k < v.cnt; k += kThreads)
    if (merges(lab[k])) merged[v.i0 + k] = 255;
}

__global__ void __launch_bounds__(kThreads) k_dilate(Ctx c) {
  __shared__ unsigned Mw[kExtWords];
  __shared__ unsigned Ow[kChunkPx / 32 + 1];
  const View v = view_of(c, blockIdx.x);
  const uint8_t* merged = c.merged + v.win.off;
  uint8_t* tmp = c.tmp + v.win.off;
  for (int i = threadIdx.x; i < kExtWords; i += kThreads) Mw[i] = 0u;
  __syncthreads();
  const Halo hl = halo_of(v);
  const int ew = hl.ew;
  const int gap = v.rw - ew;
  const uint8_t* src = merged + size_t(hl.ystart) * v.rw + hl.xs;
  for (int e0 = 0; e0 < hl.ext; e0 += kThreads) {
    const int e = e0 + threadIdx.x;
    const int row = gap == 0 ? 0 : (e >= ew) + (e >= 2 * ew);
    const unsigned m = __ballot_sync(0xffffffffu, e < hl.ext && src[e + row * gap] != 0);
    if ((threadIdx.x & 31) == 0 && e < hl.ext) Mw[e >> 5] = m;
  }
  __syncthreads();
  const DivW dv = make_div(ew, 3 * (kChunkPx + 2) + 1);
  for (int w = threadIdx.x; w * 32 < v.cnt; w += kThreads) {
    const int p = w * 32 + hl.off;
    int ye, xe;
    divmod(p, dv, ye, xe);
    unsigned rs, re;
    row_ends(hl.xs + xe, v.rw, rs, re);
    unsigned o = bits_from(Mw, p) | bits_from(Mw, p - ew) | bits_from(Mw, p + ew);
    o |= (bits_from(Mw, p - 1) | bits_from(Mw, p - ew - 1) | bits_from(Mw, p + ew - 1)) & ~rs;
    o |= (bits_from(Mw, p + 1) | bits_from(Mw, p - ew + 1) | bits_from(Mw, p + ew + 1)) & ~re;
    Ow[w] = o;
  }
  __syncthreads();
  for (int k = threadIdx.x; k < v.cnt; k += kThreads) tmp[v.i0 + k] = ((Ow[k >> 5] >> (k & 31)) & 1u) ? 255 : 0;
}
__global__ void __launch_bounds__(kThreads) k_or(Ctx c) {
  const View v = view_of(c, blockIdx.x);
  const uint8_t* merged = c.merged + v.win.off;
  const DivW dv = make_div(v.rw, v.rw * v.rh);
  constexpr int U = 8;
  for (int k0 = 0; k0 < v.cnt; k0 += kThreads * U) {
    uint8_t mg[U];
#pragma unroll
    for (int u = 0; u < U; ++u) {
      const int k = k0 + u * kThreads + threadIdx.x;
      mg[u] = k < v.cnt ? merged[v.i0 + k] : 0;
    }
#pragma unroll
    for (int u = 0; u < U; ++u) {
      if (!mg[u]) continue;
      int y, x;
      divmod(v.i0 + k0 + u * kThreads + threadIdx.x, dv, y, x);
      const size_t gp = size_t(v.win.page_off) + size_t(v.win.y1 + y) * v.win.pitch + v.win.x1 + x;
      atomicOr(&c.out_all[gp >> 2], 0xffu << (8 * (gp & 3)));
    }
  }
}

}

size_t refine_mk_state_bytes(int n_wins) { return (size_t(n_wins) * sizeof(WinState) + 255) / 256 * 256; }
size_t refine_scratch_bytes(size_t total_px, size_t n_chunks) {
  return total_px * (4 + 16 + 2 + 2 + 4) + n_chunks * 4 + 4096;
}

cudaError_t refine_mk_launch(const uint8_t* d_img, const uint8_t* d_mask, const RefineWin* d_wins, int n_wins,
                             const RefineChunk* d_chunks, int n_chunks, int n_multi_chunks, void* d_state, size_t total_px,
                             void* scratch, int refine_mode, uint8_t* d_out, cudaStream_t s) {
  if (n_wins <= 0 || n_chunks <= 0) return cudaSuccess;
  Ctx c;
  c.img_all = d_img; c.mask_all = d_mask; c.out_all = reinterpret_cast<uint32_t*>(d_out);
  c.wins = d_wins;
  c.chunks = d_chunks;
  c.st = static_cast<WinState*>(d_state);
  c.mode = refine_mode;
  char* p = static_cast<char*>(scratch);
  c.P = reinterpret_cast<int*>(p); p += total_px * 4;
  c.acc = reinterpret_cast<int*>(p); p += total_px * 16;
  c.lab = reinterpret_cast<uint16_t*>(p); p += total_px * 2;
  c.roots = reinterpret_cast<uint16_t*>(p); p += total_px * 2;
  c.nroots = reinterpret_cast<int*>(p); p += size_t(n_chunks) * 4;
  c.grey = reinterpret_cast<uint8_t*>(p); p += total_px;
  c.predm = reinterpret_cast<uint8_t*>(p); p += total_px;
  c.merged = reinterpret_cast<uint8_t*>(p); p += total_px;
  c.tmp = reinterpret_cast<uint8_t*>(p);
  cudaError_t e = cudaMemsetAsync(d_state, 0, refine_mk_state_bytes(n_wins), s);
  if (e != cudaSuccess) return e;
  const unsigned g = unsigned(n_chunks);
  k_phase0<<<g, kThreads, 0, s>>>(c);
  k_decide1<<<unsigned(n_wins), kDecideThreads, 0, s>>>(c);
  k_xor<<<g, kThreads, 0, s>>>(c);
  k_decide2<<<unsigned((n_wins + 127) / 128), 128, 0, s>>>(c, n_wins);
  for (int round = 0; round < 5; ++round) {
    if (round == 4 && refine_mode == 0) {
      k_dilate<<<g, kThreads, 0, s>>>(c);
      uint8_t* t = c.merged; c.merged = c.tmp; c.tmp = t;
    }
    k_label_local<<<g, kLabelThreads, 0, s>>>(c, round);
    if (n_multi_chunks > 0) {
      k_union_border<<<unsigned(n_multi_chunks), kBorderThreads, 0, s>>>(c, round);
      k_flat1<<<unsigned(n_multi_chunks), kThreads, 0, s>>>(c, round);
    }
    if (round == 4) {
      k_top_a<<<g, kThreads, 0, s>>>(c);
      k_top_b<<<g, kThreads, 0, s>>>(c);
    }
    k_mapply<<<g, kThreads, 0, s>>>(c, round);
  }
  k_or<<<g, kThreads, 0, s>>>(c);
  return cudaGetLastError();
}

}
```

Measured before the change: 1024.

## Pack refine masks into bit planes and defer merge application into label pass

Replaces the byte-per-pixel pred/merged/tmp planes in the text-mask refinement with packed 32-bit bit planes, precomputes the six candidate threshold masks as bit planes in k_xor, and builds label inputs from those words instead of re-thresholding grey and image bytes each round. Merge decisions are now flagged in the root list, and the flagged runs are applied at the start of the next label pass (or in a new k_merge/k_or step), rather than in a separate byte-wide pass. The goal is to cut memory traffic and per-pixel work in the refinement loop. In exchange it adds run-scanning logic, extra scratch for the candidate planes, per-chunk word offsets, and more intricate halo gathering in dilate.

```diff
diff --git a/comic-text-detector_b200/csrc/engine.h b/comic-text-detector_b200/csrc/engine.h
--- a/comic-text-detector_b200/csrc/engine.h
+++ b/comic-text-detector_b200/csrc/engine.h
@@ -132,6 +132,7 @@
   std::vector<ctd::RefineWin> wins;
   std::vector<ctd::RefineChunk> chunks;
   size_t total_px = 0;
+  size_t total_words = 0;
   void add(int x1, int y1, int x2, int y2, size_t page_off, int iw, int ih);
   size_t table_bytes() const;
 };
diff --git a/comic-text-detector_b200/csrc/kernels.h b/comic-text-detector_b200/csrc/kernels.h
--- a/comic-text-detector_b200/csrc/kernels.h
+++ b/comic-text-detector_b200/csrc/kernels.h
@@ -189,7 +189,7 @@
   long long page_off;
   int pitch;
 };
-struct RefineChunk { int win, y0, x0, rows; };
+struct RefineChunk { int win, y0, x0, rows, woff; };
 constexpr int kRefineChunkPx = 8192;
 __host__ __device__ constexpr int refine_rows_per_chunk(int rw) {
   return kRefineChunkPx / rw >= 8 ? (kRefineChunkPx / rw) & ~3 : (kRefineChunkPx / rw > 0 ? kRefineChunkPx / rw : 1);
diff --git a/comic-text-detector_b200/csrc/pipeline.cu b/comic-text-detector_b200/csrc/pipeline.cu
--- a/comic-text-detector_b200/csrc/pipeline.cu
+++ b/comic-text-detector_b200/csrc/pipeline.cu
@@ -37,7 +37,11 @@
   const int rw = x2 - x1, rh = y2 - y1;
   const int rows_per = refine_rows_per_chunk(rw);
   for (int y0 = 0; y0 < rh; y0 += rows_per)
-    for (int x0 = 0; x0 < rw; x0 += kRefineChunkPx) chunks.push_back(RefineChunk{wi, y0, x0, std::min(rows_per, rh - y0)});
+    for (int x0 = 0; x0 < rw; x0 += kRefineChunkPx) {
+      const int rows = std::min(rows_per, rh - y0);
+      chunks.push_back(RefineChunk{wi, y0, x0, rows, int(total_words)});
+      total_words += (size_t(rows) * std::min(rw - x0, kRefineChunkPx) + 31) / 32;
+    }
   wins.push_back(RefineWin{x1, y1, x2, y2, (long long)total_px, (long long)page_off, iw});
   total_px = (total_px + a + 3) / 4 * 4;
 }
diff --git a/comic-text-detector_b200/csrc/refine_mk.cu b/comic-text-detector_b200/csrc/refine_mk.cu
--- a/comic-text-detector_b200/csrc/refine_mk.cu
+++ b/comic-text-detector_b200/csrc/refine_mk.cu
@@ -33,14 +33,18 @@
   int* nroots;
   int* P;
   int* acc;
-  uint8_t *grey, *predm, *merged, *tmp;
+  uint8_t* grey;
+  unsigned* cand;
+  unsigned *pred, *merged, *tmp;
+  size_t plane_words;
 };
 constexpr uint16_t kNoLabel = 0xffffu;
-static_assert(kChunkPx <= 0xffff, "a chunk-local offset fits 16 bits below kNoLabel");
+constexpr unsigned kMergeBit = 0x8000u;
+static_assert(kChunkPx <= int(kMergeBit), "a chunk-local offset fits the 15 bits below kMergeBit");
 
 struct View {
   RefineWin win;
-  int w, rw, rh, y0, x0, rows, cols, i0, cnt, aligned;
+  int w, rw, rh, y0, x0, rows, cols, i0, cnt, woff;
   const uint8_t* img;
   const uint8_t* mask;
 };
@@ -58,7 +62,7 @@
   v.cols = min(v.rw - ch.x0, kChunkPx);
   v.i0 = ch.y0 * v.rw + ch.x0;
   v.cnt = ch.rows * v.cols;
-  v.aligned = (v.i0 & 3) == 0;
+  v.woff = ch.woff;
   v.img = c.img_all + size_t(v.win.page_off) * 3;
   v.mask = c.mask_all + size_t(v.win.page_off);
   return v;
@@ -130,6 +134,31 @@
   }
 }
 
+__device__ __forceinline__ unsigned tail_mask(int w, int cnt) {
+  const int rem = cnt - 32 * w;
+  return rem >= 32 ? 0xffffffffu : (1u << rem) - 1u;
+}
+__device__ __forceinline__ unsigned row_start_bits(int x0, int rw) {
+  unsigned rs = 0u;
+  for (int j = x0 == 0 ? 0 : rw - x0; j < 32; j += rw) rs |= 1u << j;
+  return rs;
+}
+__device__ __forceinline__ int run_end(unsigned M, unsigned S, int sbit) {
+  const unsigned stop = (~M | S) & (0xfffffffeu << sbit);
+  return stop ? __ffs(stop) - 2 : 31;
+}
+__device__ __forceinline__ unsigned span_bits(int lo, int hi) {
+  return (hi == 31 ? 0xffffffffu : ((2u << hi) - 1u)) & ~((1u << lo) - 1u);
+}
+__device__ __forceinline__ unsigned copied_word(const unsigned* src, int sb, int len, int db, int d) {
+  const int r = 32 * d - db;
+  if (r <= -32 || r >= len) return 0u;
+  const int pos = sb + max(r, 0);
+  unsigned o = __funnelshift_r(src[pos >> 5], src[(pos >> 5) + 1], pos & 31);
+  if (len - max(r, 0) < 32) o &= (1u << (len - max(r, 0))) - 1u;
+  return r < 0 ? o << -r : o;
+}
+
 constexpr int kU = 4;
 constexpr int kExtWords = (3 * kChunkPx) / 32 + 4;
 static_assert(3 * (kChunkPx + 2) / 32 + 2 < kExtWords, "a row segment's halo rectangle fits the shared bit masks");
@@ -152,8 +181,7 @@
   return __funnelshift_r(M[w], M[w + 1], sft);
 }
 __device__ __forceinline__ void row_ends(int x, int rw, unsigned& rs, unsigned& re) {
-  rs = 0u;
-  for (int j = x == 0 ? 0 : rw - x; j < 32; j += rw) rs |= 1u << j;
+  rs = row_start_bits(x, rw);
   int xe = x + 32;
   if (xe >= rw) xe %= rw;
   re = (rs >> 1) | (xe == 0 ? 0x80000000u : 0u);
@@ -161,14 +189,12 @@
 __global__ void __launch_bounds__(kThreads) k_phase0(Ctx c) {
   __shared__ int sh[4][256];
   __shared__ unsigned N60[kExtWords], N127[kExtWords];
-  __shared__ unsigned F60[kChunkPx / 32 + 1], F127[kChunkPx / 32 + 1];
+  __shared__ unsigned F127[kChunkPx / 32 + 1];
   const View v = view_of(c, blockIdx.x);
   for (int i = threadIdx.x; i < 1024; i += kThreads) (&sh[0][0])[i] = 0;
   for (int i = threadIdx.x; i < kExtWords; i += kThreads) { N60[i] = 0u; N127[i] = 0u; }
   __syncthreads();
   uint8_t* grey = c.grey + v.win.off;
-  uint8_t* predm = c.predm + v.win.off;
-  uint8_t* merged = c.merged + v.win.off;
   const Halo hl = halo_of(v);
   const DivW dv = make_div(hl.ew, 3 * (kChunkPx + 2) + 1);
   for (int e0 = 0; e0 < hl.ext; e0 += kThreads) {
@@ -190,8 +216,10 @@
     divmod(p, dv, ye, xe);
     unsigned rs, re;
     row_ends(hl.xs + xe, v.rw, rs, re);
-    F60[w] = bits_from(N60, p) | bits_from(N60, p - ew) | bits_from(N60, p + ew) | (bits_from(N60, p - 1) & ~rs) |
-             (bits_from(N60, p + 1) & ~re);
+    const unsigned f60 = bits_from(N60, p) | bits_from(N60, p - ew) | bits_from(N60, p + ew) | (bits_from(N60, p - 1) & ~rs) |
+                         (bits_from(N60, p + 1) & ~re);
+    c.pred[v.woff + w] = ~f60 & tail_mask(w, v.cnt);
+    c.merged[v.woff + w] = 0u;
     F127[w] = bits_from(N127, p) | bits_from(N127, p - ew) | bits_from(N127, p + ew) |
               ((bits_from(N127, p - 1) | bits_from(N127, p - ew - 1) | bits_from(N127, p + ew - 1)) & ~rs) |
               ((bits_from(N127, p + 1) | bits_from(N127, p - ew + 1) | bits_from(N127, p + ew + 1)) & ~re);
@@ -221,8 +249,6 @@
         const int i = v.i0 + k;
         gr = (b[u] * 1868 + g[u] * 9617 + r[u] * 4899 + 8192) >> 14;
         grey[i] = (uint8_t)gr;
-        predm[i] = ((F60[k >> 5] >> (k & 31)) & 1u) ? 0 : 255;
-        merged[i] = 0;
         core = !((F127[k >> 5] >> (k & 31)) & 1u);
       }
       if (k0 + u * kThreads < v.cnt) {
@@ -335,6 +361,7 @@
 
 __global__ void __launch_bounds__(kThreads) k_xor(Ctx c) {
   __shared__ unsigned long long sx[12];
+  __shared__ unsigned Cw[6][kChunkPx / 32];
   const View v = view_of(c, blockIdx.x);
   const WinState& st = c.st[v.w];
   if (threadIdx.x < 12) sx[threadIdx.x] = 0ull;
@@ -353,7 +380,9 @@
 #pragma unroll
     for (int u = 0; u < kU; ++u) {
       const int k = k0 + u * kThreads + threadIdx.x;
-      mk[u] = -1;
+      mk[u] = -1; gr[u] = 0;
+#pragma unroll
+      for (int q = 0; q < 3; ++q) ch[u][q] = 0;
       if (k < v.cnt) {
         int y, x;
         divmod(v.i0 + k, dv, y, x);
@@ -366,14 +395,20 @@
     }
 #pragma unroll
     for (int u = 0; u < kU; ++u) {
-      if (mk[u] < 0) continue;
-      ++npx;
+      const int kb = k0 + u * kThreads + (int(threadIdx.x) & ~31);
+      if (kb >= v.cnt) continue;
+      const bool in = mk[u] >= 0;
+      npx += in;
 #pragma unroll
       for (int k = 0; k < 3; ++k) {
-        const int t = (gr[u] >= lo[k] && gr[u] <= hi[k]) ? 255 : 0;
-        pos[k] += (unsigned)(t ^ mk[u]);
-        const int t2 = ch[u][k] > ot[k] ? 255 : 0;
-        pos[3 + k] += (unsigned)(t2 ^ mk[u]);
+        const bool t = in && gr[u] >= lo[k] && gr[u] <= hi[k];
+        const bool t2 = in && ch[u][k] > ot[k];
+        if (in) {
+          pos[k] += (unsigned)((t ? 255 : 0) ^ mk[u]);
+          pos[3 + k] += (unsigned)((t2 ? 255 : 0) ^ mk[u]);
+        }
+        const unsigned b = __ballot_sync(0xffffffffu, t), b2 = __ballot_sync(0xffffffffu, t2);
+        if ((threadIdx.x & 31) == 0) { Cw[k][kb >> 5] = b; Cw[3 + k][kb >> 5] = b2; }
       }
     }
   }
@@ -392,6 +427,12 @@
   }
   __syncthreads();
   if (threadIdx.x < 12 && sx[threadIdx.x]) atomicAdd(&c.st[v.w].xs[threadIdx.x], sx[threadIdx.x]);
+  const int nw = (v.cnt + 31) >> 5;
+  for (int k = 0; k < 6; ++k) {
+    if (k < 3 && k >= ncol) continue;
+    unsigned* cw = c.cand + k * c.plane_words + v.woff;
+    for (int w = threadIdx.x; w < nw; w += kThreads) cw[w] = Cw[k][w];
+  }
 }
 
 __global__ void k_decide2(Ctx c, int n_wins) {
@@ -427,6 +468,49 @@
 }
 
 constexpr int kLabelThreads = 512;
+
+struct Source { const unsigned* words; unsigned flip; };
+__device__ __forceinline__ Source source_of(const Ctx& c, const WinState& st, const View& v, int round) {
+  if (round == 4) return Source{c.merged + v.woff, 0xffffffffu};
+  return Source{c.cand + size_t(st.proc_kind[round]) * c.plane_words + v.woff, st.proc_neg[round] ? 0xffffffffu : 0u};
+}
+
+__device__ void apply_merges(const Ctx& c, const View& v, int chunk, int round, unsigned* dec) {
+  for (int i = threadIdx.x; i < kChunkPx / 32; i += blockDim.x) dec[i] = 0u;
+  __syncthreads();
+  const uint16_t* roots = c.roots + v.win.off + v.i0;
+  const int nr = c.nroots[chunk];
+  bool any = false;
+  for (int j = threadIdx.x; j < nr; j += blockDim.x) {
+    const unsigned e = roots[j];
+    if (e & kMergeBit) { atomicOr(&dec[(e ^ kMergeBit) >> 5], 1u << (e & 31)); any = true; }
+  }
+  if (!__syncthreads_or(any)) return;
+  const uint16_t* lab = c.lab + v.win.off + v.i0;
+  const Source src = source_of(c, c.st[v.w], v, round);
+  unsigned* merged = c.merged + v.woff;
+  const DivW dv = make_div(v.rw, kChunkPx + 1);
+  for (int hw0 = 0; hw0 * 16 < v.cnt; hw0 += blockDim.x) {
+    const int hw = hw0 + threadIdx.x, w = hw >> 1;
+    unsigned add = 0u;
+    if (hw * 16 < v.cnt) {
+      const unsigned M = (src.words[w] ^ src.flip) & tail_mask(w, v.cnt);
+      if (M) {
+        int yl, x0;
+        divmod(w * 32, dv, yl, x0);
+        const unsigned S = M & (~(M << 1) | row_start_bits(x0, v.rw));
+        for (unsigned f = S & ((hw & 1) ? 0xffff0000u : 0x0000ffffu); f; f &= f - 1u) {
+          const int sbit = __ffs(f) - 1;
+          const unsigned l = lab[w * 32 + sbit];
+          if ((dec[l >> 5] >> (l & 31)) & 1u) add |= span_bits(sbit, run_end(M, S, sbit));
+        }
+      }
+    }
+    add |= __shfl_xor_sync(0xffffffffu, add, 1);
+    if (add && !(hw & 1)) merged[w] |= add;
+  }
+  __syncthreads();
+}
 
 __device__ __forceinline__ int suf_find(const int* L, int a) {
   int p = L[a];
@@ -465,6 +549,23 @@
   } while (!done);
 }
 
+#ifdef CTD_REFINE_PASS_CLOCKS
+__device__ unsigned long long g_pass_clocks[5][8];
+#define PASS_CLOCK_BEGIN() long long pass_t0 = clock64()
+#define PASS_CLOCK(pass)                                                                        \
+  do {                                                                                          \
+    __syncthreads();                                                                            \
+    if (threadIdx.x == 0) {                                                                     \
+      const long long t = clock64();                                                            \
+      atomicAdd(&g_pass_clocks[round][pass], (unsigned long long)(t - pass_t0));                \
+      pass_t0 = t;                                                                              \
+    }                                                                                           \
+  } while (0)
+#else
+#define PASS_CLOCK_BEGIN()
+#define PASS_CLOCK(pass)
+#endif
+
 __global__ void __launch_bounds__(kLabelThreads, 3) k_label_local(Ctx c, int round) {
   __shared__ int Ls[kChunkPx];
   __shared__ unsigned Mw[kChunkPx / 32 + 2];
@@ -474,7 +575,10 @@
   __shared__ int s_fg, s_nroot;
   const View v = view_of(c, blockIdx.x);
   WinState& st = c.st[v.w];
+  PASS_CLOCK_BEGIN();
+  if (round >= 1 && round <= 3 && round - 1 < st.nproc) apply_merges(c, v, blockIdx.x, round - 1, Sw);
   if (round < 4 && round >= st.nproc) return;
+  PASS_CLOCK(0);
   for (int i = threadIdx.x; i < kChunkPx / 32 + 2; i += kLabelThreads) Mw[i] = 0u;
   if (threadIdx.x == 0) { s_fg = 0; s_nroot = 0; }
   __syncthreads();
@@ -484,143 +588,29 @@
   int* acc = c.acc + 4 * v.win.off;
   const int n = v.rw * v.rh;
   int* area = acc; int* gain = acc + n; int* loss = acc + 2 * n; int* maxi = acc + 3 * n;
-  const uint8_t* grey = c.grey + v.win.off;
-  const uint8_t* merged = c.merged + v.win.off;
-  const uint8_t* predm = c.predm + v.win.off;
-  int kind = 0, neg = 0, lo = 0, hi = 0, ot = 0;
-  if (round < 4) {
-    kind = st.proc_kind[round]; neg = st.proc_neg[round];
-    if (kind < 3) { lo = st.lo[kind]; hi = st.hi[kind]; } else ot = st.otsu_t[kind - 3];
-  }
-  const int lane = threadIdx.x & 31;
   const DivW dv = make_div(v.rw, kChunkPx + 1);
-  constexpr int kIt = kChunkPx / kLabelThreads;
-  if (v.aligned) {
-    const uint32_t* mg32 = reinterpret_cast<const uint32_t*>(merged + v.i0);
-    const uint32_t* pd32 = reinterpret_cast<const uint32_t*>(predm + v.i0);
-    const uint32_t* gr32 = reinterpret_cast<const uint32_t*>(grey + v.i0);
-    const int sh = 4 * (lane & 7);
-    const unsigned grp = 0xffu << (8 * (lane >> 3));
-#pragma unroll 1
-    for (int it = 0; it < kChunkPx / (4 * kLabelThreads); ++it) {
-      if (it * 4 * kLabelThreads >= v.cnt) break;
-      const int k = 4 * (it * kLabelThreads + int(threadIdx.x));
-      unsigned fg4 = 0u, g4 = 0u, b4 = 0u;
-      if (k < v.cnt) {
-        const unsigned m4 = mg32[k >> 2], p4 = pd32[k >> 2];
-        unsigned s4 = m4;
-        if (round < 4) {
-          if (kind < 3) {
-            s4 = gr32[k >> 2];
-          } else {
-            s4 = 0u;
-#pragma unroll
-            for (int j = 0; j < 4; ++j) {
-              if (k + j < v.cnt) {
-                int yl, x;
-                divmod(k + j, dv, yl, x);
-                s4 |= unsigned(v.img[(size_t(v.win.y1 + v.y0 + yl) * v.win.pitch + v.win.x1 + v.x0 + x) * 3 + (kind - 3)]) << (8 * j);
-              }
-            }
-          }
-        }
-#pragma unroll
-        for (int j = 0; j < 4; ++j) {
-          if (k + j < v.cnt) {
-            const int sbv = int((s4 >> (8 * j)) & 0xffu), mb = int((m4 >> (8 * j)) & 0xffu), pb = int((p4 >> (8 * j)) & 0xffu);
-            bool fg;
-            if (round == 4) {
-              fg = sbv == 0;
-            } else {
-              const bool t = kind < 3 ? (sbv >= lo && sbv <= hi) : (sbv > ot);
-              fg = neg ? !t : t;
-            }
-            const bool un = fg && mb == 0;
-            fg4 |= unsigned(fg) << j;
-            g4 |= unsigned(un && pb != 0) << j;
-            b4 |= unsigned(un && pb == 0) << j;
-          }
-        }
-      }
-      const unsigned M = __reduce_or_sync(grp, fg4 << sh), G = __reduce_or_sync(grp, g4 << sh), B = __reduce_or_sync(grp, b4 << sh);
-      if ((lane & 7) == 0) { const int w = k >> 5; Mw[w] = M; Gw[w] = G; Bw[w] = B; }
-    }
-    __syncthreads();
-    for (int w = threadIdx.x; w * 32 < v.cnt; w += kLabelThreads) {
-      const unsigned M = Mw[w];
+  {
+    const Source src = source_of(c, st, v, round);
+    const unsigned* mgw = c.merged + v.woff;
+    const unsigned* pdw = c.pred + v.woff;
+    for (int hw = threadIdx.x; hw * 16 < v.cnt; hw += kLabelThreads) {
+      const int w = hw >> 1;
+      const unsigned M = (src.words[w] ^ src.flip) & tail_mask(w, v.cnt);
       int yl, x0;
       divmod(w * 32, dv, yl, x0);
-      unsigned rs = 0u;
-      for (int j = x0 == 0 ? 0 : v.rw - x0; j < 32; j += v.rw) rs |= 1u << j;
-      const unsigned S = M & (~(M << 1) | rs);
-      Sw[w] = S;
-      unsigned f = S;
-      while (f) {
+      const unsigned S = M & (~(M << 1) | row_start_bits(x0, v.rw));
+      if (!(hw & 1)) {
+        const unsigned un = M & ~mgw[w], pd = pdw[w];
+        Mw[w] = M; Sw[w] = S; Gw[w] = un & pd; Bw[w] = un & ~pd;
+      }
+      for (unsigned f = S & ((hw & 1) ? 0xffff0000u : 0x0000ffffu); f; f &= f - 1u) {
         const int k = w * 32 + __ffs(f) - 1;
-        f &= f - 1u;
         Ls[k] = k;
       }
     }
-  } else {
-    constexpr int kB = 4;
-    int xrun, xstep;
-    {
-      int q;
-      divmod(int(threadIdx.x), dv, q, xrun);
-      divmod(kLabelThreads, dv, q, xstep);
-    }
-  #pragma unroll 1
-    for (int ub = 0; ub < kIt; ub += kB) {
-      if (ub * kLabelThreads >= v.cnt) break;
-      int raw[kB], mg[kB], pd[kB];
-  #pragma unroll
-      for (int u = 0; u < kB; ++u) {
-        const int k = (ub + u) * kLabelThreads + threadIdx.x;
-        raw[u] = 0; mg[u] = 1; pd[u] = 0;
-        if (k < v.cnt) {
-          const int i = v.i0 + k;
-          mg[u] = merged[i];
-          pd[u] = predm[i];
-          if (round == 4) raw[u] = mg[u];
-          else if (kind < 3) raw[u] = grey[i];
-          else {
-            int yl, x;
-            divmod(k, dv, yl, x);
-            raw[u] = v.img[(size_t(v.win.y1 + v.y0 + yl) * v.win.pitch + v.win.x1 + v.x0 + x) * 3 + (kind - 3)];
-          }
-        }
-      }
-  #pragma unroll
-      for (int u = 0; u < kB; ++u) {
-        const int k0 = (ub + u) * kLabelThreads;
-        if (k0 >= v.cnt) break;
-        const int k = k0 + threadIdx.x;
-        const bool in = k < v.cnt;
-        int sv = 0;
-        const int x = xrun;
-        xrun += xstep;
-        if (xrun >= v.rw) xrun -= v.rw;
-        if (in) {
-          if (round == 4) {
-            sv = raw[u] ? 0 : 255;
-          } else {
-            const int tv = kind < 3 ? ((raw[u] >= lo && raw[u] <= hi) ? 255 : 0) : (raw[u] > ot ? 255 : 0);
-            sv = neg ? 255 - tv : tv;
-          }
-        }
-        const bool fg = in && sv != 0;
-        const bool un = fg && mg[u] == 0;
-        const unsigned m = __ballot_sync(0xffffffffu, fg);
-        const unsigned gb = __ballot_sync(0xffffffffu, un && pd[u] != 0);
-        const unsigned lb = __ballot_sync(0xffffffffu, un && pd[u] == 0);
-        const bool starts = fg && (lane == 0 || x == 0 || !((m >> (lane - 1)) & 1u));
-        const unsigned sb = __ballot_sync(0xffffffffu, starts);
-        if (lane == 0) { Mw[k >> 5] = m; Sw[k >> 5] = sb; Gw[k >> 5] = gb; Bw[k >> 5] = lb; }
-        if (starts) Ls[k] = k;
-      }
-    }
-  }
-  __syncthreads();
+  }
+  __syncthreads();
+  PASS_CLOCK(1);
   auto start_of = [&](int pos) -> int {
     return (pos & ~31) + 31 - __clz(Sw[pos >> 5] & (0xffffffffu >> (31 - (pos & 31))));
   };
@@ -638,8 +628,7 @@
     const int k0 = w * 32;
     int yl, x0;
     divmod(k0, dv, yl, x0);
-    unsigned rs = 0u;
-    for (int j = x0 == 0 ? 0 : v.rw - x0; j < 32; j += v.rw) rs |= 1u << j;
+    const unsigned rs = row_start_bits(x0, v.rw);
     int xe = x0 + 32;
     if (xe >= v.rw) xe %= v.rw;
     const unsigned re = (rs >> 1) | (xe == 0 ? 0x80000000u : 0u);
@@ -669,6 +658,7 @@
     }
   }
   __syncthreads();
+  PASS_CLOCK(3);
   int fgc = 0;
   for (int hw = threadIdx.x; hw * 16 < v.cnt; hw += kLabelThreads) {
     const unsigned half = (hw & 1) ? 0xffff0000u : 0x0000ffffu;
@@ -691,7 +681,7 @@
   }
   if (round == 4) {
     for (int o = 16; o > 0; o >>= 1) fgc += __shfl_down_sync(0xffffffffu, fgc, o);
-    if (lane == 0 && fgc) atomicAdd(&s_fg, fgc);
+    if ((threadIdx.x & 31) == 0 && fgc) atomicAdd(&s_fg, fgc);
   }
   __syncthreads();
   if (threadIdx.x == 0) {
@@ -699,8 +689,10 @@
     const int a0 = v.cnt - s_fg;
     if (round == 4 && a0) atomicAdd(&st.area0, a0);
   }
+  PASS_CLOCK(4);
   for (int k = threadIdx.x; k < v.cnt; k += kLabelThreads)
     lab[k] = ((Mw[k >> 5] >> (k & 31)) & 1u) ? uint16_t(Ls[start_of(k)]) : kNoLabel;
+  PASS_CLOCK(5);
   for (int hw = threadIdx.x; hw * 16 < v.cnt; hw += kLabelThreads) {
     const int w = hw >> 1;
     const unsigned M = Mw[w], S = Sw[w];
@@ -711,9 +703,8 @@
     while (f) {
       const int sbit = __ffs(f) - 1;
       f &= f - 1u;
-      const unsigned stop = (~M | S) & (0xfffffffeu << sbit);
-      const int e = stop ? __ffs(stop) - 2 : 31;
-      const unsigned rm = (e == 31 ? 0xffffffffu : ((2u << e) - 1u)) & ~((1u << sbit) - 1u);
+      const int e = run_end(M, S, sbit);
+      const unsigned rm = span_bits(sbit, e);
       const int gi = v.i0 + Ls[k0 + sbit];
       atomicAdd(&area[gi], __popc(rm));
       atomicMax(&maxi[gi], v.i0 + k0 + e);
@@ -722,6 +713,7 @@
       if (l_) atomicAdd(&loss[gi], l_);
     }
   }
+  PASS_CLOCK(6);
 }
 constexpr int kBorderThreads = 256;
 __global__ void __launch_bounds__(kBorderThreads) k_union_border(Ctx c, int round) {
@@ -810,20 +802,17 @@
     if (m2 >= 0) atomicMax(&st.max2, m2);
   }
 }
-__global__ void __launch_bounds__(kThreads) k_mapply(Ctx c, int round) {
+__global__ void __launch_bounds__(kThreads) k_decide_roots(Ctx c, int round) {
   const View v = view_of(c, blockIdx.x);
   const WinState& st = c.st[v.w];
   if (round < 4 && round >= st.nproc) return;
-  const uint16_t* lab = c.lab + v.win.off + v.i0;
   const int* P = c.P + v.win.off;
-  uint8_t* merged = c.merged + v.win.off;
   const int* acc = c.acc + 4 * v.win.off;
   const int n = v.rw * v.rh;
   const int* area = acc; const int* gain = acc + n; const int* loss = acc + 2 * n; const int* maxi = acc + 3 * n;
   const int second = st.cnt1 >= 2 ? st.max1 : st.max2;
   const int thresh = second >= 0 ? second : st.max1;
-  __shared__ uint8_t dec[kChunkPx];
-  const uint16_t* roots = c.roots + v.win.off + v.i0;
+  uint16_t* roots = c.roots + v.win.off + v.i0;
   const int nr = c.nroots[blockIdx.x];
   for (int j = threadIdx.x; j < nr; j += kThreads) {
     const int cl = roots[j];
@@ -836,47 +825,60 @@
     } else {
       ok = a < thresh;
     }
-    dec[cl] = ok && gain[g] > loss[g];
-  }
-  __syncthreads();
-  auto merges = [&](unsigned l) { return l != kNoLabel && dec[l]; };
-  int k_tail = 0;
-  if (v.aligned) {
-    const uint2* lab4 = reinterpret_cast<const uint2*>(lab);
-    uint32_t* mg32 = reinterpret_cast<uint32_t*>(merged + v.i0);
-    const int n4 = v.cnt >> 2;
-    for (int q = threadIdx.x; q < n4; q += kThreads) {
-      const uint2 l4 = lab4[q];
-      const unsigned m = (merges(l4.x & 0xffffu) ? 0xffu : 0u) | (merges(l4.x >> 16) ? 0xff00u : 0u) |
-                         (merges(l4.y & 0xffffu) ? 0xff0000u : 0u) | (merges(l4.y >> 16) ? 0xff000000u : 0u);
-      if (m) mg32[q] |= m;
-    }
-    k_tail = n4 << 2;
-  }
-  for (int k = k_tail + threadIdx.x; k < v.cnt; k += kThreads)
-    if (merges(lab[k])) merged[v.i0 + k] = 255;
+    if (ok && gain[g] > loss[g]) roots[j] = uint16_t(cl | kMergeBit);
+  }
+}
+__global__ void __launch_bounds__(kThreads) k_merge(Ctx c, int round) {
+  __shared__ unsigned dec[kChunkPx / 32];
+  const View v = view_of(c, blockIdx.x);
+  if (round >= c.st[v.w].nproc) return;
+  apply_merges(c, v, blockIdx.x, round, dec);
 }
 
 __global__ void __launch_bounds__(kThreads) k_dilate(Ctx c) {
   __shared__ unsigned Mw[kExtWords];
-  __shared__ unsigned Ow[kChunkPx / 32 + 1];
-  const View v = view_of(c, blockIdx.x);
-  const uint8_t* merged = c.merged + v.win.off;
-  uint8_t* tmp = c.tmp + v.win.off;
+  const View v = view_of(c, blockIdx.x);
   for (int i = threadIdx.x; i < kExtWords; i += kThreads) Mw[i] = 0u;
   __syncthreads();
   const Halo hl = halo_of(v);
   const int ew = hl.ew;
-  const int gap = v.rw - ew;
-  const uint8_t* src = merged + size_t(hl.ystart) * v.rw + hl.xs;
-  for (int e0 = 0; e0 < hl.ext; e0 += kThreads) {
+  const DivW dv = make_div(ew, 3 * (kChunkPx + 2) + 1);
+  const bool seg = v.rw > kChunkPx;
+  const int nseg = (v.rw + kChunkPx - 1) / kChunkPx;
+  const int rows_up = seg ? 1 : refine_rows_per_chunk(v.rw);
+  if (!seg) {
+    const bool up = v.y0 > 0, down = v.y0 + v.rows < v.rh;
+    const unsigned* mu = up ? c.merged + c.chunks[blockIdx.x - 1].woff : nullptr;
+    const unsigned* md = down ? c.merged + c.chunks[blockIdx.x + 1].woff : nullptr;
+    for (int d = threadIdx.x; d * 32 < hl.ext; d += kThreads) {
+      unsigned m = copied_word(c.merged + v.woff, 0, v.cnt, hl.off, d);
+      if (up) m |= copied_word(mu, (rows_up - 1) * v.rw, v.rw, 0, d);
+      if (down) m |= copied_word(md, 0, v.rw, hl.off + v.cnt, d);
+      Mw[d] = m;
+    }
+  }
+  for (int e0 = 0; seg && e0 < hl.ext; e0 += kThreads) {
     const int e = e0 + threadIdx.x;
-    const int row = gap == 0 ? 0 : (e >= ew) + (e >= 2 * ew);
-    const unsigned m = __ballot_sync(0xffffffffu, e < hl.ext && src[e + row * gap] != 0);
+    bool bit = false;
+    if (e < hl.ext) {
+      int ye, xe;
+      divmod(e, dv, ye, xe);
+      const int y = hl.ystart + ye, x = hl.xs + xe;
+      const int dy = y < v.y0 ? -1 : (y >= v.y0 + v.rows ? 1 : 0);
+      int ch = int(blockIdx.x) + dy * (seg ? nseg : 1), k;
+      if (seg) {
+        ch += x / kChunkPx - v.x0 / kChunkPx;
+        k = x % kChunkPx;
+      } else {
+        k = (dy < 0 ? rows_up - 1 : (dy > 0 ? 0 : y - v.y0)) * v.rw + x;
+      }
+      const int wo = ch == int(blockIdx.x) ? v.woff : c.chunks[ch].woff;
+      bit = (c.merged[wo + (k >> 5)] >> (k & 31)) & 1u;
+    }
+    const unsigned m = __ballot_sync(0xffffffffu, bit);
     if ((threadIdx.x & 31) == 0 && e < hl.ext) Mw[e >> 5] = m;
   }
   __syncthreads();
-  const DivW dv = make_div(ew, 3 * (kChunkPx + 2) + 1);
   for (int w = threadIdx.x; w * 32 < v.cnt; w += kThreads) {
     const int p = w * 32 + hl.off;
     int ye, xe;
@@ -886,39 +888,39 @@
     unsigned o = bits_from(Mw, p) | bits_from(Mw, p - ew) | bits_from(Mw, p + ew);
     o |= (bits_from(Mw, p - 1) | bits_from(Mw, p - ew - 1) | bits_from(Mw, p + ew - 1)) & ~rs;
     o |= (bits_from(Mw, p + 1) | bits_from(Mw, p - ew + 1) | bits_from(Mw, p + ew + 1)) & ~re;
-    Ow[w] = o;
-  }
-  __syncthreads();
-  for (int k = threadIdx.x; k < v.cnt; k += kThreads) tmp[v.i0 + k] = ((Ow[k >> 5] >> (k & 31)) & 1u) ? 255 : 0;
+    c.tmp[v.woff + w] = o & tail_mask(w, v.cnt);
+  }
 }
 __global__ void __launch_bounds__(kThreads) k_or(Ctx c) {
-  const View v = view_of(c, blockIdx.x);
-  const uint8_t* merged = c.merged + v.win.off;
+  __shared__ unsigned dec[kChunkPx / 32];
+  const View v = view_of(c, blockIdx.x);
+  apply_merges(c, v, blockIdx.x, 4, dec);
+  const unsigned* merged = c.merged + v.woff;
   const DivW dv = make_div(v.rw, v.rw * v.rh);
-  constexpr int U = 8;
-  for (int k0 = 0; k0 < v.cnt; k0 += kThreads * U) {
-    uint8_t mg[U];
-#pragma unroll
-    for (int u = 0; u < U; ++u) {
-      const int k = k0 + u * kThreads + threadIdx.x;
-      mg[u] = k < v.cnt ? merged[v.i0 + k] : 0;
-    }
-#pragma unroll
-    for (int u = 0; u < U; ++u) {
-      if (!mg[u]) continue;
-      int y, x;
-      divmod(v.i0 + k0 + u * kThreads + threadIdx.x, dv, y, x);
-      const size_t gp = size_t(v.win.page_off) + size_t(v.win.y1 + y) * v.win.pitch + v.win.x1 + x;
-      atomicOr(&c.out_all[gp >> 2], 0xffu << (8 * (gp & 3)));
-    }
-  }
-}
-
-}
+  for (int k = threadIdx.x; k < v.cnt; k += kThreads) {
+    if (!((merged[k >> 5] >> (k & 31)) & 1u)) continue;
+    int y, x;
+    divmod(v.i0 + k, dv, y, x);
+    const size_t gp = size_t(v.win.page_off) + size_t(v.win.y1 + y) * v.win.pitch + v.win.x1 + x;
+    atomicOr(&c.out_all[gp >> 2], 0xffu << (8 * (gp & 3)));
+  }
+}
+
+}
+
+#ifdef CTD_REFINE_PASS_CLOCKS
+extern "C" __attribute__((visibility("default"))) int ctd_refine_pass_clocks(unsigned long long* out) {
+  static const unsigned long long zero[5 * 8] = {};
+  cudaError_t e = cudaMemcpyFromSymbol(out, g_pass_clocks, sizeof(zero));
+  if (e == cudaSuccess) e = cudaMemcpyToSymbol(g_pass_clocks, zero, sizeof(zero));
+  return int(e);
+}
+#endif
 
 size_t refine_mk_state_bytes(int n_wins) { return (size_t(n_wins) * sizeof(WinState) + 255) / 256 * 256; }
+static size_t plane_words(size_t total_px, size_t n_chunks) { return total_px / 32 + n_chunks + 1; }
 size_t refine_scratch_bytes(size_t total_px, size_t n_chunks) {
-  return total_px * (4 + 16 + 2 + 2 + 4) + n_chunks * 4 + 4096;
+  return total_px * (4 + 16 + 2 + 2 + 1) + n_chunks * 4 + 9 * 4 * plane_words(total_px, n_chunks) + 4096;
 }
 
 cudaError_t refine_mk_launch(const uint8_t* d_img, const uint8_t* d_mask, const RefineWin* d_wins, int n_wins,
@@ -938,9 +940,11 @@
   c.roots = reinterpret_cast<uint16_t*>(p); p += total_px * 2;
   c.nroots = reinterpret_cast<int*>(p); p += size_t(n_chunks) * 4;
   c.grey = reinterpret_cast<uint8_t*>(p); p += total_px;
-  c.predm = reinterpret_cast<uint8_t*>(p); p += total_px;
-  c.merged = reinterpret_cast<uint8_t*>(p); p += total_px;
-  c.tmp = reinterpret_cast<uint8_t*>(p);
+  c.plane_words = plane_words(total_px, size_t(n_chunks));
+  c.cand = reinterpret_cast<unsigned*>(p); p += 6 * 4 * c.plane_words;
+  c.pred = reinterpret_cast<unsigned*>(p); p += 4 * c.plane_words;
+  c.merged = reinterpret_cast<unsigned*>(p); p += 4 * c.plane_words;
+  c.tmp = reinterpret_cast<unsigned*>(p);
   cudaError_t e = cudaMemsetAsync(d_state, 0, refine_mk_state_bytes(n_wins), s);
   if (e != cudaSuccess) return e;
   const unsigned g = unsigned(n_chunks);
@@ -949,9 +953,10 @@
   k_xor<<<g, kThreads, 0, s>>>(c);
   k_decide2<<<unsigned((n_wins + 127) / 128), 128, 0, s>>>(c, n_wins);
   for (int round = 0; round < 5; ++round) {
+    if (round == 4) k_merge<<<g, kThreads, 0, s>>>(c, 3);
     if (round == 4 && refine_mode == 0) {
       k_dilate<<<g, kThreads, 0, s>>>(c);
-      uint8_t* t = c.merged; c.merged = c.tmp; c.tmp = t;
+      unsigned* t = c.merged; c.merged = c.tmp; c.tmp = t;
     }
     k_label_local<<<g, kLabelThreads, 0, s>>>(c, round);
     if (n_multi_chunks > 0) {
@@ -962,7 +967,7 @@
       k_top_a<<<g, kThreads, 0, s>>>(c);
       k_top_b<<<g, kThreads, 0, s>>>(c);
     }
-    k_mapply<<<g, kThreads, 0, s>>>(c, round);
+    k_decide_roots<<<g, kThreads, 0, s>>>(c, round);
   }
   k_or<<<g, kThreads, 0, s>>>(c);
   return cudaGetLastError();
```

Result: faster. 1090, median of 6 (+6.5%).
